# 0xPolygonZero/proof-protocol-decoder

Measured on AMD Instinct MI355X. Metric: txn-proofs/sec (whole node), 256-txn synthetic block, higher is better.
Workload: dtype u64 (Goldilocks field)

## Files before the change

proof_protocol_decoder_amd/csrc/gl.hpp:

```cpp
#pragma once
#include <cstdint>
#include <hip/hip_runtime.h>

#define GL_HD __host__ __device__ __forceinline__

namespace gl {

constexpr uint64_t P = 0xFFFFFFFF00000001ULL;
constexpr uint64_t EPS = 0xFFFFFFFFULL;
constexpr uint64_t GENERATOR = 7;
constexpr uint64_t TWO_ADIC_ROOT = 1753635133440165772ULL;
constexpr uint64_t W = 7;

#if defined(__HIP__)
namespace cc {
typedef uint64_t mask;
__device__ __forceinline__ uint64_t mad_co(uint32_t a, uint32_t b, uint64_t c, mask& co) {
  uint64_t d;
  asm("v_mad_u64_u32 %0, %1, %2, %3, %4" : "=v"(d), "=s"(co) : "v"(a), "v"(b), "v"(c));
  return d;
}
__device__ __forceinline__ uint64_t mad_eps_co(uint32_t a, uint64_t c, mask& co) {
  uint64_t d;
  asm("v_mad_u64_u32 %0, %1, %2, -1, %3" : "=v"(d), "=s"(co) : "v"(a), "v"(c));
  return d;
}
__device__ __forceinline__ uint32_t add_co(uint32_t a, uint32_t b, mask& co) {
  uint32_t d;
  asm("v_add_co_u32_e64 %0, %1, %2, %3" : "=v"(d), "=s"(co) : "v"(a), "v"(b));
  return d;
}
__device__ __forceinline__ uint32_t addc_co(uint32_t a, uint32_t b, mask ci, mask& co) {
  uint32_t d;
  asm("s_nop 1\n\tv_addc_co_u32_e64 %0, %1, %2, %3, %4" : "=v"(d), "=s"(co) : "v"(a), "v"(b), "s"(ci));
  return d;
}
__device__ __forceinline__ uint32_t addc0_co(uint32_t a, mask ci, mask& co) {
  uint32_t d;
  asm("s_nop 1\n\tv_addc_co_u32_e64 %0, %1, %2, 0, %3" : "=v"(d), "=s"(co) : "v"(a), "s"(ci));
  return d;
}
__device__ __forceinline__ uint32_t sub_co(uint32_t a, uint32_t b, mask& co) {
  uint32_t d;
  asm("v_sub_co_u32_e64 %0, %1, %2, %3" : "=v"(d), "=s"(co) : "v"(a), "v"(b));
  return d;
}
__device__ __forceinline__ uint32_t subb_co(uint32_t a, uint32_t b, mask ci, mask& co) {
  uint32_t d;
  asm("s_nop 1\n\tv_subb_co_u32_e64 %0, %1, %2, %3, %4" : "=v"(d), "=s"(co) : "v"(a), "v"(b), "s"(ci));
  return d;
}
__device__ __forceinline__ uint32_t subb0_co(uint32_t a, mask ci, mask& co) {
  uint32_t d;
  asm("s_nop 1\n\tv_subbrev_co_u32_e64 %0, %1, 0, %2, %3" : "=v"(d), "=s"(co) : "v"(a), "s"(ci));
  return d;
}
__device__ __forceinline__ uint32_t sel_eps(mask m) {
  uint32_t d;
  asm("s_nop 1\n\tv_cndmask_b32_e64 %0, 0, -1, %1" : "=v"(d) : "s"(m));
  return d;
}
__device__ __forceinline__ uint64_t mk64(uint32_t lo, uint32_t hi) { return ((uint64_t)hi << 32) | lo; }
#include "gl_cc.inc"
}
#endif
GL_HD uint64_t canon(uint64_t a) {
  return a >= P ? a - P : a;
}

GL_HD uint64_t add(uint64_t a, uint64_t b) {
  uint64_t s = a + b;
  return s < b ? s + EPS : s;
}
GL_HD uint64_t sub(uint64_t a, uint64_t b) {
  uint64_t d = a - b;
  return a < b ? d - EPS : d;
}
GL_HD uint64_t addc(uint64_t a, uint64_t b) {
  uint64_t s = a + b;
  return (s < a || s >= P) ? s - P : s;
}
GL_HD uint64_t subc(uint64_t a, uint64_t b) {
  return a >= b ? a - b : a + (P - b);
}
GL_HD uint64_t negc(uint64_t a) {
  return a ? P - a : 0;
}

GL_HD uint64_t reduce128(uint64_t lo, uint64_t hi) {
  uint64_t hh = hi >> 32, hl = hi & EPS;
  uint64_t t0 = lo - hh;
  if (lo < hh) t0 -= EPS;
  uint64_t t1 = (hl << 32) - hl;
  uint64_t r = t0 + t1;
  return r < t1 ? r + EPS : r;
}

GL_HD void mul_wide(uint64_t a, uint64_t b, uint64_t& lo, uint64_t& hi) {
#if defined(__HIP_DEVICE_COMPILE__)
  uint32_t a0 = (uint32_t)a, a1 = (uint32_t)(a >> 32), b0 = (uint32_t)b, b1 = (uint32_t)(b >> 32);
  uint64_t p00 = (uint64_t)a0 * b0;
  uint64_t mid = (uint64_t)a0 * b1 + (p00 >> 32);
  uint64_t mid2 = (uint64_t)a1 * b0 + (uint32_t)mid;
  hi = (uint64_t)a1 * b1 + (mid >> 32) + (mid2 >> 32);
  lo = (mid2 << 32) | (uint32_t)p00;
#else
  unsigned __int128 x = (unsigned __int128)a * b;
  lo = (uint64_t)x;
  hi = (uint64_t)(x >> 64);
#endif
}

GL_HD uint64_t mul(uint64_t a, uint64_t b) {
#if defined(__HIP_DEVICE_COMPILE__)
  const uint32_t a0 = (uint32_t)a, a1 = (uint32_t)(a >> 32), b0 = (uint32_t)b, b1 = (uint32_t)(b >> 32);
  cc::mask C, c1, c2, c3, cx, bw, bw2, b3;
  const uint64_t P = (uint64_t)a0 * b0;
  const uint64_t M = cc::mad_co(a1, b0, (uint64_t)a0 * b1, C);
  const uint64_t Q = (uint64_t)a1 * b1;
  const uint32_t p1 = cc::add_co((uint32_t)(P >> 32), (uint32_t)M, c1);
  const uint32_t S = cc::addc_co((uint32_t)(M >> 32), (uint32_t)Q, c1, c2);
  const uint32_t K = cc::addc0_co((uint32_t)(Q >> 32), C, cx);
  const uint64_t V = cc::mad_eps_co(S, cc::mk64((uint32_t)P, p1), c3);
  const uint32_t t0 = cc::subb0_co((uint32_t)V, c3, b3);
  const uint32_t t1 = cc::addc0_co((uint32_t)(V >> 32), c3 & ~b3, cx);
  const uint32_t u0 = cc::subb_co(t0, K, c2, bw);
  const uint32_t u1 = cc::subb0_co(t1, bw, bw2);
  const uint32_t r0 = cc::addc0_co(u0, bw2, b3);
  const uint32_t r1 = cc::subb0_co(u1, bw2 & ~b3, cx);
  return cc::mk64(r0, r1);
#else
  uint64_t lo, hi;
  mul_wide(a, b, lo, hi);
  return reduce128(lo, hi);
#endif
}
#if defined(__HIP__)
template <int N>
__device__ __forceinline__ void mul_n(const uint64_t (&a)[N], const uint64_t (&b)[N], uint64_t (&r)[N]) {
  static_assert(N == 3 || N == 4, "groups of 3 or 4");
  uint32_t a1[N], b0[N], t0[N], t1[N], m0[N], m1[N], q0[N], q1[N];
  uint64_t P[N], M[N], Q[N];
  cc::mask C[N], c1[N], c2[N], c3[N], bw[N], bw2[N], b3[N];
#pragma unroll
  for (int i = 0; i < N; i++) {
    const uint32_t a0 = (uint32_t)a[i], b1 = (uint32_t)(b[i] >> 32);
    a1[i] = (uint32_t)(a[i] >> 32);
    b0[i] = (uint32_t)b[i];
    P[i] = (uint64_t)a0 * b0[i];
    M[i] = (uint64_t)a0 * b1;
    Q[i] = (uint64_t)a1[i] * b1;
  }
  cc::mad_co(M, C, a1, b0);
#pragma unroll
  for (int i = 0; i < N; i++) {
    t0[i] = (uint32_t)P[i]; t1[i] = (uint32_t)(P[i] >> 32); m0[i] = (uint32_t)M[i]; m1[i] = (uint32_t)(M[i] >> 32);
    q0[i] = (uint32_t)Q[i]; q1[i] = (uint32_t)(Q[i] >> 32);
  }
  cc::add_co(t1, c1, m0);
  cc::addc_co(m1, c2, q0, c1);
  cc::addc0_cv(q1, C);
#pragma unroll
  for (int i = 0; i < N; i++) P[i] = cc::mk64(t0[i], t1[i]);
  cc::mad_eps_co(P, c3, m1);
#pragma unroll
  for (int i = 0; i < N; i++) { t0[i] = (uint32_t)P[i]; t1[i] = (uint32_t)(P[i] >> 32); }
  cc::subb0_co(t0, b3, c3);
#pragma unroll
  for (int i = 0; i < N; i++) c3[i] &= ~b3[i];
  cc::addc0_cv(t1, c3);
  cc::subb_co(t0, bw, q1, c2);
  cc::subb0_co(t1, bw2, bw);
  cc::addc0_co(t0, b3, bw2);
#pragma unroll
  for (int i = 0; i < N; i++) bw2[i] &= ~b3[i];
  cc::subb0_cv(t1, bw2);
#pragma unroll
  for (int i = 0; i < N; i++) r[i] = cc::mk64(t0[i], t1[i]);
}
#endif
#if defined(__HIP__)
template <int N>
__device__ __forceinline__ void add_n(const uint64_t (&a)[N], const uint64_t (&b)[N], uint64_t (&r)[N]) {
  uint32_t al[N], ah[N], bl[N], bh[N], lo[N], hi[N];
  cc::mask c1[N], c2[N], c3[N];
#pragma unroll
  for (int i = 0; i < N; i++) {
    al[i] = (uint32_t)a[i]; ah[i] = (uint32_t)(a[i] >> 32); bl[i] = (uint32_t)b[i]; bh[i] = (uint32_t)(b[i] >> 32);
  }
  cc::add_co_o(lo, c1, al, bl);
  cc::addc_co_o(hi, c2, ah, bh, c1);
  cc::subb0_co(lo, c3, c2);
#pragma unroll
  for (int i = 0; i < N; i++) c2[i] &= ~c3[i];
  cc::addc0_cv(hi, c2);
#pragma unroll
  for (int i = 0; i < N; i++) r[i] = cc::mk64(lo[i], hi[i]);
}
template <int N>
__device__ __forceinline__ void sub_n(const uint64_t (&a)[N], const uint64_t (&b)[N], uint64_t (&r)[N]) {
  uint32_t al[N], ah[N], bl[N], bh[N], lo[N], hi[N];
  cc::mask b1[N], b2[N], b3[N];
#pragma unroll
  for (int i = 0; i < N; i++) {
    al[i] = (uint32_t)a[i]; ah[i] = (uint32_t)(a[i] >> 32); bl[i] = (uint32_t)b[i]; bh[i] = (uint32_t)(b[i] >> 32);
  }
  cc::sub_co_o(lo, b1, al, bl);
  cc::subb_co_o(hi, b2, ah, bh, b1);
  cc::addc0_co(lo, b3, b2);
#pragma unroll
  for (int i = 0; i < N; i++) b2[i] &= ~b3[i];
  cc::subb0_cv(hi, b2);
#pragma unroll
  for (int i = 0; i < N; i++) r[i] = cc::mk64(lo[i], hi[i]);
}
template <int N>
__device__ __forceinline__ void canon_n(uint64_t (&a)[N]) {
  uint32_t lo[N], hi[N], tl[N], th[N];
  cc::mask k[N], c[N];
#pragma unroll
  for (int i = 0; i < N; i++) {
    lo[i] = (uint32_t)a[i]; hi[i] = (uint32_t)(a[i] >> 32);
  }
  cc::add_m1_co_o(tl, k, lo);
  cc::addc0_co_o(th, c, hi, k);
  cc::sel(lo, tl, c);
  cc::sel(hi, th, c);
#pragma unroll
  for (int i = 0; i < N; i++) a[i] = cc::mk64(lo[i], hi[i]);
}
#endif
#if defined(__HIP__)
struct DotAcc {
  uint64_t p, m, q;
  uint32_t cp, cm, cq;
};
__device__ __forceinline__ DotAcc dot_zero() { return DotAcc{0, 0, 0, 0, 0, 0}; }
__device__ __forceinline__ void dot_mad4(DotAcc (&acc)[4], const uint64_t (&a)[4], const uint64_t (&b)[4]) {
  uint32_t a0[4], a1[4], b0[4], b1[4], cnt[4];
  uint64_t col[4];
  cc::mask c[4], cx[4];
#pragma unroll
  for (int i = 0; i < 4; i++) {
    a0[i] = (uint32_t)a[i]; a1[i] = (uint32_t)(a[i] >> 32); b0[i] = (uint32_t)b[i]; b1[i] = (uint32_t)(b[i] >> 32);
  }
#define BPG_DOT_COL(COL, CNT, X, Y)                                  \
  _Pragma("unroll") for (int i = 0; i < 4; i++) { col[i] = acc[i].COL; cnt[i] = acc[i].CNT; } \
  cc::mad_co(col, c, X, Y);                                           \
  cc::addc0_co(cnt, cx, c);                                           \
  _Pragma("unroll") for (int i = 0; i < 4; i++) { acc[i].COL = col[i]; acc[i].CNT = cnt[i]; }
  BPG_DOT_COL(p, cp, a0, b0)
  BPG_DOT_COL(m, cm, a0, b1)
  BPG_DOT_COL(m, cm, a1, b0)
  BPG_DOT_COL(q, cq, a1, b1)
#undef BPG_DOT_COL
}
GL_HD uint64_t mulc(uint64_t a, uint64_t b);
GL_HD uint64_t addc(uint64_t a, uint64_t b);
__device__ __forceinline__ uint64_t dot_reduce(const DotAcc& d) {
  uint64_t r = canon(d.p);
  r = addc(r, mulc(d.m, (uint64_t)1 << 32));
  r = addc(r, mulc(d.q, EPS));
  r = addc(r, mulc(d.cp, EPS));
  r = subc(r, canon((uint64_t)d.cm));
  r = subc(r, mulc(d.cq, (uint64_t)1 << 32));
  return r;
}
#endif
GL_HD uint64_t sqr(uint64_t a) { return mul(a, a); }
GL_HD uint64_t mulc(uint64_t a, uint64_t b) { return canon(mul(a, b)); }

GL_HD uint64_t pow(uint64_t a, uint64_t e) {
  uint64_t r = 1;
  while (e) {
    if (e & 1) r = mulc(r, a);
    a = mulc(a, a);
    e >>= 1;
  }
  return r;
}
GL_HD uint64_t inv(uint64_t a) {
  auto sq_n = [](uint64_t x, int n) {
    for (int i = 0; i < n; i++) x = mul(x, x);
    return x;
  };
  const uint64_t e1 = a;
  const uint64_t e2 = mul(sq_n(e1, 1), e1);
  const uint64_t e3 = mul(sq_n(e2, 1), e1);
  const uint64_t e6 = mul(sq_n(e3, 3), e3);
  const uint64_t e12 = mul(sq_n(e6, 6), e6);
  const uint64_t e24 = mul(sq_n(e12, 12), e12);
  const uint64_t e30 = mul(sq_n(e24, 6), e6);
  const uint64_t e31 = mul(sq_n(e30, 1), e1);
  const uint64_t hi = sq_n(e31, 1);
  const uint64_t lo = mul(hi, a);
  return mulc(sq_n(hi, 32), lo);
}
GL_HD uint64_t root(unsigned k) {
  uint64_t r = TWO_ADIC_ROOT;
  for (unsigned i = k; i < 32; i++) r = mulc(r, r);
  return r;
}

struct Ext {
  uint64_t c0, c1;
};
GL_HD Ext ext(uint64_t a, uint64_t b = 0) { return Ext{a, b}; }
GL_HD bool eq(Ext a, Ext b) { return a.c0 == b.c0 && a.c1 == b.c1; }
GL_HD Ext add(Ext a, Ext b) { return Ext{addc(a.c0, b.c0), addc(a.c1, b.c1)}; }
GL_HD Ext sub(Ext a, Ext b) { return Ext{subc(a.c0, b.c0), subc(a.c1, b.c1)}; }
GL_HD uint64_t mul7(uint64_t x) {
  const uint64_t p = (uint64_t)(uint32_t)x * 7u;
  const uint64_t m = (x >> 32) * 7u + (p >> 32);
  const uint64_t u = (m << 32) | (uint32_t)p;
  const uint64_t t = u + (m >> 32) * EPS;
  return t < u ? t + EPS : t;
}
GL_HD Ext mul(Ext a, Ext b) {
#if defined(__HIP_DEVICE_COMPILE__)
  const uint64_t x[4] = {a.c0, a.c1, a.c0, a.c1}, y[4] = {b.c0, b.c1, b.c1, b.c0};
  uint64_t r[4];
  mul_n<4>(x, y, r);
  return Ext{addc(canon(r[0]), canon(mul7(r[1]))), addc(canon(r[2]), canon(r[3]))};
#else
  uint64_t c0 = addc(mulc(a.c0, b.c0), mulc(W, mulc(a.c1, b.c1)));
  uint64_t c1 = addc(mulc(a.c0, b.c1), mulc(a.c1, b.c0));
  return Ext{c0, c1};
#endif
}
GL_HD Ext scale(Ext a, uint64_t s) { return Ext{mulc(a.c0, s), mulc(a.c1, s)}; }
GL_HD Ext pow(Ext a, uint64_t e) {
  Ext r = ext(1);
  while (e) {
    if (e & 1) r = mul(r, a);
    a = mul(a, a);
    e >>= 1;
  }
  return r;
}
GL_HD Ext inv(Ext a) {
  uint64_t n = subc(mulc(a.c0, a.c0), mulc(W, mulc(a.c1, a.c1)));
  uint64_t ni = inv(n);
  return Ext{mulc(a.c0, ni), mulc(negc(a.c1), ni)};
}

GL_HD uint32_t bitrev(uint32_t x, unsigned bits) {
#if defined(__HIP_DEVICE_COMPILE__)
  return bits ? (__brev(x) >> (32 - bits)) : 0;
#else
  uint32_t r = 0;
  for (unsigned i = 0; i < bits; i++) r |= ((x >> i) & 1u) << (bits - 1 - i);
  return r;
#endif
}

}
```

proof_protocol_decoder_amd/csrc/gl_cc.inc:

```
__device__ __forceinline__ void mad_co(uint64_t (&x)[3], mask (&co)[3], const uint32_t (&a)[3], const uint32_t (&b)[3]) {
  asm("v_mad_u64_u32 %0, %3, %6, %9, %0\n\tv_mad_u64_u32 %1, %4, %7, %10, %1\n\tv_mad_u64_u32 %2, %5, %8, %11, %2"
      : "+v"(x[0]), "+v"(x[1]), "+v"(x[2]), "=&s"(co[0]), "=&s"(co[1]), "=&s"(co[2])
      : "v"(a[0]), "v"(a[1]), "v"(a[2]), "v"(b[0]), "v"(b[1]), "v"(b[2]));
}
__device__ __forceinline__ void mad_eps_co(uint64_t (&x)[3], mask (&co)[3], const uint32_t (&a)[3]) {
  asm("v_mad_u64_u32 %0, %3, %6, -1, %0\n\tv_mad_u64_u32 %1, %4, %7, -1, %1\n\tv_mad_u64_u32 %2, %5, %8, -1, %2"
      : "+v"(x[0]), "+v"(x[1]), "+v"(x[2]), "=&s"(co[0]), "=&s"(co[1]), "=&s"(co[2])
      : "v"(a[0]), "v"(a[1]), "v"(a[2]));
}
__device__ __forceinline__ void add_co(uint32_t (&x)[3], mask (&co)[3], const uint32_t (&b)[3]) {
  asm("v_add_co_u32_e64 %0, %3, %0, %6\n\tv_add_co_u32_e64 %1, %4, %1, %7\n\tv_add_co_u32_e64 %2, %5, %2, %8"
      : "+v"(x[0]), "+v"(x[1]), "+v"(x[2]), "=&s"(co[0]), "=&s"(co[1]), "=&s"(co[2])
      : "v"(b[0]), "v"(b[1]), "v"(b[2]));
}
__device__ __forceinline__ void addc_co(uint32_t (&x)[3], mask (&co)[3], const uint32_t (&b)[3], const mask (&ci)[3]) {
  asm("v_addc_co_u32_e64 %0, %3, %0, %6, %9\n\tv_addc_co_u32_e64 %1, %4, %1, %7, %10\n\tv_addc_co_u32_e64 %2, %5, %2, %8, %11"
      : "+v"(x[0]), "+v"(x[1]), "+v"(x[2]), "=&s"(co[0]), "=&s"(co[1]), "=&s"(co[2])
      : "v"(b[0]), "v"(b[1]), "v"(b[2]), "s"(ci[0]), "s"(ci[1]), "s"(ci[2]));
}
__device__ __forceinline__ void addc0_co(uint32_t (&x)[3], mask (&co)[3], const mask (&ci)[3]) {
  asm("v_addc_co_u32_e64 %0, %3, %0, 0, %6\n\tv_addc_co_u32_e64 %1, %4, %1, 0, %7\n\tv_addc_co_u32_e64 %2, %5, %2, 0, %8"
      : "+v"(x[0]), "+v"(x[1]), "+v"(x[2]), "=&s"(co[0]), "=&s"(co[1]), "=&s"(co[2])
      : "s"(ci[0]), "s"(ci[1]), "s"(ci[2]));
}
__device__ __forceinline__ void sub_co(uint32_t (&x)[3], mask (&co)[3], const uint32_t (&b)[3]) {
  asm("v_sub_co_u32_e64 %0, %3, %0, %6\n\tv_sub_co_u32_e64 %1, %4, %1, %7\n\tv_sub_co_u32_e64 %2, %5, %2, %8"
      : "+v"(x[0]), "+v"(x[1]), "+v"(x[2]), "=&s"(co[0]), "=&s"(co[1]), "=&s"(co[2])
      : "v"(b[0]), "v"(b[1]), "v"(b[2]));
}
__device__ __forceinline__ void subb_co(uint32_t (&x)[3], mask (&co)[3], const uint32_t (&b)[3], const mask (&ci)[3]) {
  asm("v_subb_co_u32_e64 %0, %3, %0, %6, %9\n\tv_subb_co_u32_e64 %1, %4, %1, %7, %10\n\tv_subb_co_u32_e64 %2, %5, %2, %8, %11"
      : "+v"(x[0]), "+v"(x[1]), "+v"(x[2]), "=&s"(co[0]), "=&s"(co[1]), "=&s"(co[2])
      : "v"(b[0]), "v"(b[1]), "v"(b[2]), "s"(ci[0]), "s"(ci[1]), "s"(ci[2]));
}
__device__ __forceinline__ void subb0_co(uint32_t (&x)[3], mask (&co)[3], const mask (&ci)[3]) {
  asm("v_subbrev_co_u32_e64 %0, %3, 0, %0, %6\n\tv_subbrev_co_u32_e64 %1, %4, 0, %1, %7\n\tv_subbrev_co_u32_e64 %2, %5, 0, %2, %8"
      : "+v"(x[0]), "+v"(x[1]), "+v"(x[2]), "=&s"(co[0]), "=&s"(co[1]), "=&s"(co[2])
      : "s"(ci[0]), "s"(ci[1]), "s"(ci[2]));
}
__device__ __forceinline__ void add_m1_co(uint32_t (&x)[3], mask (&co)[3]) {
  asm("v_add_co_u32_e64 %0, %3, %0, -1\n\tv_add_co_u32_e64 %1, %4, %1, -1\n\tv_add_co_u32_e64 %2, %5, %2, -1"
      : "+v"(x[0]), "+v"(x[1]), "+v"(x[2]), "=&s"(co[0]), "=&s"(co[1]), "=&s"(co[2])
      : );
}
__device__ __forceinline__ void sel(uint32_t (&x)[3], const uint32_t (&b)[3], const mask (&ci)[3]) {
  asm("v_cndmask_b32_e64 %0, %0, %3, %6\n\tv_cndmask_b32_e64 %1, %1, %4, %7\n\tv_cndmask_b32_e64 %2, %2, %5, %8"
      : "+v"(x[0]), "+v"(x[1]), "+v"(x[2])
      : "v"(b[0]), "v"(b[1]), "v"(b[2]), "s"(ci[0]), "s"(ci[1]), "s"(ci[2]));
}
__device__ __forceinline__ void sel_eps(uint32_t (&x)[3], const mask (&ci)[3]) {
  asm("v_cndmask_b32_e64 %0, 0, -1, %3\n\tv_cndmask_b32_e64 %1, 0, -1, %4\n\tv_cndmask_b32_e64 %2, 0, -1, %5"
      : "=&v"(x[0]), "=&v"(x[1]), "=&v"(x[2])
      : "s"(ci[0]), "s"(ci[1]), "s"(ci[2]));
}
__device__ __forceinline__ void addc0_cv(uint32_t (&x)[3], const mask (&ci)[3]) {
  asm("v_addc_co_u32_e64 %0, vcc, %0, 0, %3\n\tv_addc_co_u32_e64 %1, vcc, %1, 0, %4\n\tv_addc_co_u32_e64 %2, vcc, %2, 0, %5"
      : "+v"(x[0]), "+v"(x[1]), "+v"(x[2])
      : "s"(ci[0]), "s"(ci[1]), "s"(ci[2]) : "vcc");
}
__device__ __forceinline__ void addc_cv(uint32_t (&x)[3], const uint32_t (&b)[3], const mask (&ci)[3]) {
  asm("v_addc_co_u32_e64 %0, vcc, %0, %3, %6\n\tv_addc_co_u32_e64 %1, vcc, %1, %4, %7\n\tv_addc_co_u32_e64 %2, vcc, %2, %5, %8"
      : "+v"(x[0]), "+v"(x[1]), "+v"(x[2])
      : "v"(b[0]), "v"(b[1]), "v"(b[2]), "s"(ci[0]), "s"(ci[1]), "s"(ci[2]) : "vcc");
}
__device__ __forceinline__ void subb0_cv(uint32_t (&x)[3], const mask (&ci)[3]) {
  asm("v_subbrev_co_u32_e64 %0, vcc, 0, %0, %3\n\tv_subbrev_co_u32_e64 %1, vcc, 0, %1, %4\n\tv_subbrev_co_u32_e64 %2, vcc, 0, %2, %5"
      : "+v"(x[0]), "+v"(x[1]), "+v"(x[2])
      : "s"(ci[0]), "s"(ci[1]), "s"(ci[2]) : "vcc");
}
__device__ __forceinline__ void mad_eps_cv(uint64_t (&x)[3], const uint32_t (&a)[3]) {
  asm("v_mad_u64_u32 %0, vcc, %3, -1, %0\n\tv_mad_u64_u32 %1, vcc, %4, -1, %1\n\tv_mad_u64_u32 %2, vcc, %5, -1, %2"
      : "+v"(x[0]), "+v"(x[1]), "+v"(x[2])
      : "v"(a[0]), "v"(a[1]), "v"(a[2]) : "vcc");
}
__device__ __forceinline__ void sel_one(uint32_t (&x)[3], const mask (&ci)[3]) {
  asm("v_cndmask_b32_e64 %0, %0, 1, %3\n\tv_cndmask_b32_e64 %1, %1, 1, %4\n\tv_cndmask_b32_e64 %2, %2, 1, %5"
      : "+v"(x[0]), "+v"(x[1]), "+v"(x[2])
      : "s"(ci[0]), "s"(ci[1]), "s"(ci[2]));
}
__device__ __forceinline__ void add_co_o(uint32_t (&x)[3], mask (&co)[3], const uint32_t (&a)[3], const uint32_t (&b)[3]) {
  asm("v_add_co_u32_e64 %0, %3, %6, %9\n\tv_add_co_u32_e64 %1, %4, %7, %10\n\tv_add_co_u32_e64 %2, %5, %8, %11"
      : "=&v"(x[0]), "=&v"(x[1]), "=&v"(x[2]), "=&s"(co[0]), "=&s"(co[1]), "=&s"(co[2])
      : "v"(a[0]), "v"(a[1]), "v"(a[2]), "v"(b[0]), "v"(b[1]), "v"(b[2]));
}
__device__ __forceinline__ void addc_co_o(uint32_t (&x)[3], mask (&co)[3], const uint32_t (&a)[3], const uint32_t (&b)[3], const mask (&ci)[3]) {
  asm("v_addc_co_u32_e64 %0, %3, %6, %9, %12\n\tv_addc_co_u32_e64 %1, %4, %7, %10, %13\n\tv_addc_co_u32_e64 %2, %5, %8, %11, %14"
      : "=&v"(x[0]), "=&v"(x[1]), "=&v"(x[2]), "=&s"(co[0]), "=&s"(co[1]), "=&s"(co[2])
      : "v"(a[0]), "v"(a[1]), "v"(a[2]), "v"(b[0]), "v"(b[1]), "v"(b[2]), "s"(ci[0]), "s"(ci[1]), "s"(ci[2]));
}
__device__ __forceinline__ void sub_co_o(uint32_t (&x)[3], mask (&co)[3], const uint32_t (&a)[3], const uint32_t (&b)[3]) {
  asm("v_sub_co_u32_e64 %0, %3, %6, %9\n\tv_sub_co_u32_e64 %1, %4, %7, %10\n\tv_sub_co_u32_e64 %2, %5, %8, %11"
      : "=&v"(x[0]), "=&v"(x[1]), "=&v"(x[2]), "=&s"(co[0]), "=&s"(co[1]), "=&s"(co[2])
      : "v"(a[0]), "v"(a[1]), "v"(a[2]), "v"(b[0]), "v"(b[1]), "v"(b[2]));
}
__device__ __forceinline__ void subb_co_o(uint32_t (&x)[3], mask (&co)[3], const uint32_t (&a)[3], const uint32_t (&b)[3], const mask (&ci)[3]) {
  asm("v_subb_co_u32_e64 %0, %3, %6, %9, %12\n\tv_subb_co_u32_e64 %1, %4, %7, %10, %13\n\tv_subb_co_u32_e64 %2, %5, %8, %11, %14"
      : "=&v"(x[0]), "=&v"(x[1]), "=&v"(x[2]), "=&s"(co[0]), "=&s"(co[1]), "=&s"(co[2])
      : "v"(a[0]), "v"(a[1]), "v"(a[2]), "v"(b[0]), "v"(b[1]), "v"(b[2]), "s"(ci[0]), "s"(ci[1]), "s"(ci[2]));
}
__device__ __forceinline__ void add_m1_co_o(uint32_t (&x)[3], mask (&co)[3], const uint32_t (&a)[3]) {
  asm("v_add_co_u32_e64 %0, %3, %6, -1\n\tv_add_co_u32_e64 %1, %4, %7, -1\n\tv_add_co_u32_e64 %2, %5, %8, -1"
      : "=&v"(x[0]), "=&v"(x[1]), "=&v"(x[2]), "=&s"(co[0]), "=&s"(co[1]), "=&s"(co[2])
      : "v"(a[0]), "v"(a[1]), "v"(a[2]));
}
__device__ __forceinline__ void addc0_co_o(uint32_t (&x)[3], mask (&co)[3], const uint32_t (&a)[3], const mask (&ci)[3]) {
  asm("v_addc_co_u32_e64 %0, %3, %6, 0, %9\n\tv_addc_co_u32_e64 %1, %4, %7, 0, %10\n\tv_addc_co_u32_e64 %2, %5, %8, 0, %11"
      : "=&v"(x[0]), "=&v"(x[1]), "=&v"(x[2]), "=&s"(co[0]), "=&s"(co[1]), "=&s"(co[2])
      : "v"(a[0]), "v"(a[1]), "v"(a[2]), "s"(ci[0]), "s"(ci[1]), "s"(ci[2]));
}
__device__ __forceinline__ void mad_co(uint64_t (&x)[4], mask (&co)[4], const uint32_t (&a)[4], const uint32_t (&b)[4]) {
  asm("v_mad_u64_u32 %0, %4, %8, %12, %0\n\tv_mad_u64_u32 %1, %5, %9, %13, %1\n\tv_mad_u64_u32 %2, %6, %10, %14, %2\n\tv_mad_u64_u32 %3, %7, %11, %15, %3"
      : "+v"(x[0]), "+v"(x[1]), "+v"(x[2]), "+v"(x[3]), "=&s"(co[0]), "=&s"(co[1]), "=&s"(co[2]), "=&s"(co[3])
      : "v"(a[0]), "v"(a[1]), "v"(a[2]), "v"(a[3]), "v"(b[0]), "v"(b[1]), "v"(b[2]), "v"(b[3]));
}
__device__ __forceinline__ void mad_eps_co(uint64_t (&x)[4], mask (&co)[4], const uint32_t (&a)[4]) {
  asm("v_mad_u64_u32 %0, %4, %8, -1, %0\n\tv_mad_u64_u32 %1, %5, %9, -1, %1\n\tv_mad_u64_u32 %2, %6, %10, -1, %2\n\tv_mad_u64_u32 %3, %7, %11, -1, %3"
      : "+v"(x[0]), "+v"(x[1]), "+v"(x[2]), "+v"(x[3]), "=&s"(co[0]), "=&s"(co[1]), "=&s"(co[2]), "=&s"(co[3])
      : "v"(a[0]), "v"(a[1]), "v"(a[2]), "v"(a[3]));
}
__device__ __forceinline__ void add_co(uint32_t (&x)[4], mask (&co)[4], const uint32_t (&b)[4]) {
  asm("v_add_co_u32_e64 %0, %4, %0, %8\n\tv_add_co_u32_e64 %1, %5, %1, %9\n\tv_add_co_u32_e64 %2, %6, %2, %10\n\tv_add_co_u32_e64 %3, %7, %3, %11"
      : "+v"(x[0]), "+v"(x[1]), "+v"(x[2]), "+v"(x[3]), "=&s"(co[0]), "=&s"(co[1]), "=&s"(co[2]), "=&s"(co[3])
      : "v"(b[0]), "v"(b[1]), "v"(b[2]), "v"(b[3]));
}
__device__ __forceinline__ void addc_co(uint32_t (&x)[4], mask (&co)[4], const uint32_t (&b)[4], const mask (&ci)[4]) {
  asm("v_addc_co_u32_e64 %0, %4, %0, %8, %12\n\tv_addc_co_u32_e64 %1, %5, %1, %9, %13\n\tv_addc_co_u32_e64 %2, %6, %2, %10, %14\n\tv_addc_co_u32_e64 %3, %7, %3, %11, %15"
      : "+v"(x[0]), "+v"(x[1]), "+v"(x[2]), "+v"(x[3]), "=&s"(co[0]), "=&s"(co[1]), "=&s"(co[2]), "=&s"(co[3])
      : "v"(b[0]), "v"(b[1]), "v"(b[2]), "v"(b[3]), "s"(ci[0]), "s"(ci[1]), "s"(ci[2]), "s"(ci[3]));
}
__device__ __forceinline__ void addc0_co(uint32_t (&x)[4], mask (&co)[4], const mask (&ci)[4]) {
  asm("v_addc_co_u32_e64 %0, %4, %0, 0, %8\n\tv_addc_co_u32_e64 %1, %5, %1, 0, %9\n\tv_addc_co_u32_e64 %2, %6, %2, 0, %10\n\tv_addc_co_u32_e64 %3, %7, %3, 0, %11"
      : "+v"(x[0]), "+v"(x[1]), "+v"(x[2]), "+v"(x[3]), "=&s"(co[0]), "=&s"(co[1]), "=&s"(co[2]), "=&s"(co[3])
      : "s"(ci[0]), "s"(ci[1]), "s"(ci[2]), "s"(ci[3]));
}
__device__ __forceinline__ void sub_co(uint32_t (&x)[4], mask (&co)[4], const uint32_t (&b)[4]) {
  asm("v_sub_co_u32_e64 %0, %4, %0, %8\n\tv_sub_co_u32_e64 %1, %5, %1, %9\n\tv_sub_co_u32_e64 %2, %6, %2, %10\n\tv_sub_co_u32_e64 %3, %7, %3, %11"
      : "+v"(x[0]), "+v"(x[1]), "+v"(x[2]), "+v"(x[3]), "=&s"(co[0]), "=&s"(co[1]), "=&s"(co[2]), "=&s"(co[3])
      : "v"(b[0]), "v"(b[1]), "v"(b[2]), "v"(b[3]));
}
__device__ __forceinline__ void subb_co(uint32_t (&x)[4], mask (&co)[4], const uint32_t (&b)[4], const mask (&ci)[4]) {
  asm("v_subb_co_u32_e64 %0, %4, %0, %8, %12\n\tv_subb_co_u32_e64 %1, %5, %1, %9, %13\n\tv_subb_co_u32_e64 %2, %6, %2, %10, %14\n\tv_subb_co_u32_e64 %3, %7, %3, %11, %15"
      : "+v"(x[0]), "+v"(x[1]), "+v"(x[2]), "+v"(x[3]), "=&s"(co[0]), "=&s"(co[1]), "=&s"(co[2]), "=&s"(co[3])
      : "v"(b[0]), "v"(b[1]), "v"(b[2]), "v"(b[3]), "s"(ci[0]), "s"(ci[1]), "s"(ci[2]), "s"(ci[3]));
}
__device__ __forceinline__ void subb0_co(uint32_t (&x)[4], mask (&co)[4], const mask (&ci)[4]) {
  asm("v_subbrev_co_u32_e64 %0, %4, 0, %0, %8\n\tv_subbrev_co_u32_e64 %1, %5, 0, %1, %9\n\tv_subbrev_co_u32_e64 %2, %6, 0, %2, %10\n\tv_subbrev_co_u32_e64 %3, %7, 0, %3, %11"
      : "+v"(x[0]), "+v"(x[1]), "+v"(x[2]), "+v"(x[3]), "=&s"(co[0]), "=&s"(co[1]), "=&s"(co[2]), "=&s"(co[3])
      : "s"(ci[0]), "s"(ci[1]), "s"(ci[2]), "s"(ci[3]));
}
__device__ __forceinline__ void add_m1_co(uint32_t (&x)[4], mask (&co)[4]) {
  asm("v_add_co_u32_e64 %0, %4, %0, -1\n\tv_add_co_u32_e64 %1, %5, %1, -1\n\tv_add_co_u32_e64 %2, %6, %2, -1\n\tv_add_co_u32_e64 %3, %7, %3, -1"
      : "+v"(x[0]), "+v"(x[1]), "+v"(x[2]), "+v"(x[3]), "=&s"(co[0]), "=&s"(co[1]), "=&s"(co[2]), "=&s"(co[3])
      : );
}
__device__ __forceinline__ void sel(uint32_t (&x)[4], const uint32_t (&b)[4], const mask (&ci)[4]) {
  asm("v_cndmask_b32_e64 %0, %0, %4, %8\n\tv_cndmask_b32_e64 %1, %1, %5, %9\n\tv_cndmask_b32_e64 %2, %2, %6, %10\n\tv_cndmask_b32_e64 %3, %3, %7, %11"
      : "+v"(x[0]), "+v"(x[1]), "+v"(x[2]), "+v"(x[3])
      : "v"(b[0]), "v"(b[1]), "v"(b[2]), "v"(b[3]), "s"(ci[0]), "s"(ci[1]), "s"(ci[2]), "s"(ci[3]));
}
__device__ __forceinline__ void sel_eps(uint32_t (&x)[4], const mask (&ci)[4]) {
  asm("v_cndmask_b32_e64 %0, 0, -1, %4\n\tv_cndmask_b32_e64 %1, 0, -1, %5\n\tv_cndmask_b32_e64 %2, 0, -1, %6\n\tv_cndmask_b32_e64 %3, 0, -1, %7"
      : "=&v"(x[0]), "=&v"(x[1]), "=&v"(x[2]), "=&v"(x[3])
      : "s"(ci[0]), "s"(ci[1]), "s"(ci[2]), "s"(ci[3]));
}
__device__ __forceinline__ void addc0_cv(uint32_t (&x)[4], const mask (&ci)[4]) {
  asm("v_addc_co_u32_e64 %0, vcc, %0, 0, %4\n\tv_addc_co_u32_e64 %1, vcc, %1, 0, %5\n\tv_addc_co_u32_e64 %2, vcc, %2, 0, %6\n\tv_addc_co_u32_e64 %3, vcc, %3, 0, %7"
      : "+v"(x[0]), "+v"(x[1]), "+v"(x[2]), "+v"(x[3])
      : "s"(ci[0]), "s"(ci[1]), "s"(ci[2]), "s"(ci[3]) : "vcc");
}
__device__ __forceinline__ void addc_cv(uint32_t (&x)[4], const uint32_t (&b)[4], const mask (&ci)[4]) {
  asm("v_addc_co_u32_e64 %0, vcc, %0, %4, %8\n\tv_addc_co_u32_e64 %1, vcc, %1, %5, %9\n\tv_addc_co_u32_e64 %2, vcc, %2, %6, %10\n\tv_addc_co_u32_e64 %3, vcc, %3, %7, %11"
      : "+v"(x[0]), "+v"(x[1]), "+v"(x[2]), "+v"(x[3])
      : "v"(b[0]), "v"(b[1]), "v"(b[2]), "v"(b[3]), "s"(ci[0]), "s"(ci[1]), "s"(ci[2]), "s"(ci[3]) : "vcc");
}
__device__ __forceinline__ void subb0_cv(uint32_t (&x)[4], const mask (&ci)[4]) {
  asm("v_subbrev_co_u32_e64 %0, vcc, 0, %0, %4\n\tv_subbrev_co_u32_e64 %1, vcc, 0, %1, %5\n\tv_subbrev_co_u32_e64 %2, vcc, 0, %2, %6\n\tv_subbrev_co_u32_e64 %3, vcc, 0, %3, %7"
      : "+v"(x[0]), "+v"(x[1]), "+v"(x[2]), "+v"(x[3])
      : "s"(ci[0]), "s"(ci[1]), "s"(ci[2]), "s"(ci[3]) : "vcc");
}
__device__ __forceinline__ void mad_eps_cv(uint64_t (&x)[4], const uint32_t (&a)[4]) {
  asm("v_mad_u64_u32 %0, vcc, %4, -1, %0\n\tv_mad_u64_u32 %1, vcc, %5, -1, %1\n\tv_mad_u64_u32 %2, vcc, %6, -1, %2\n\tv_mad_u64_u32 %3, vcc, %7, -1, %3"
      : "+v"(x[0]), "+v"(x[1]), "+v"(x[2]), "+v"(x[3])
      : "v"(a[0]), "v"(a[1]), "v"(a[2]), "v"(a[3]) : "vcc");
}
__device__ __forceinline__ void sel_one(uint32_t (&x)[4], const mask (&ci)[4]) {
  asm("v_cndmask_b32_e64 %0, %0, 1, %4\n\tv_cndmask_b32_e64 %1, %1, 1, %5\n\tv_cndmask_b32_e64 %2, %2, 1, %6\n\tv_cndmask_b32_e64 %3, %3, 1, %7"
      : "+v"(x[0]), "+v"(x[1]), "+v"(x[2]), "+v"(x[3])
      : "s"(ci[0]), "s"(ci[1]), "s"(ci[2]), "s"(ci[3]));
}
__device__ __forceinline__ void add_co_o(uint32_t (&x)[4], mask (&co)[4], const uint32_t (&a)[4], const uint32_t (&b)[4]) {
  asm("v_add_co_u32_e64 %0, %4, %8, %12\n\tv_add_co_u32_e64 %1, %5, %9, %13\n\tv_add_co_u32_e64 %2, %6, %10, %14\n\tv_add_co_u32_e64 %3, %7, %11, %15"
      : "=&v"(x[0]), "=&v"(x[1]), "=&v"(x[2]), "=&v"(x[3]), "=&s"(co[0]), "=&s"(co[1]), "=&s"(co[2]), "=&s"(co[3])
      : "v"(a[0]), "v"(a[1]), "v"(a[2]), "v"(a[3]), "v"(b[0]), "v"(b[1]), "v"(b[2]), "v"(b[3]));
}
__device__ __forceinline__ void addc_co_o(uint32_t (&x)[4], mask (&co)[4], const uint32_t (&a)[4], const uint32_t (&b)[4], const mask (&ci)[4]) {
  asm("v_addc_co_u32_e64 %0, %4, %8, %12, %16\n\tv_addc_co_u32_e64 %1, %5, %9, %13, %17\n\tv_addc_co_u32_e64 %2, %6, %10, %14, %18\n\tv_addc_co_u32_e64 %3, %7, %11, %15, %19"
      : "=&v"(x[0]), "=&v"(x[1]), "=&v"(x[2]), "=&v"(x[3]), "=&s"(co[0]), "=&s"(co[1]), "=&s"(co[2]), "=&s"(co[3])
      : "v"(a[0]), "v"(a[1]), "v"(a[2]), "v"(a[3]), "v"(b[0]), "v"(b[1]), "v"(b[2]), "v"(b[3]), "s"(ci[0]), "s"(ci[1]), "s"(ci[2]), "s"(ci[3]));
}
__device__ __forceinline__ void sub_co_o(uint32_t (&x)[4], mask (&co)[4], const uint32_t (&a)[4], const uint32_t (&b)[4]) {
  asm("v_sub_co_u32_e64 %0, %4, %8, %12\n\tv_sub_co_u32_e64 %1, %5, %9, %13\n\tv_sub_co_u32_e64 %2, %6, %10, %14\n\tv_sub_co_u32_e64 %3, %7, %11, %15"
      : "=&v"(x[0]), "=&v"(x[1]), "=&v"(x[2]), "=&v"(x[3]), "=&s"(co[0]), "=&s"(co[1]), "=&s"(co[2]), "=&s"(co[3])
      : "v"(a[0]), "v"(a[1]), "v"(a[2]), "v"(a[3]), "v"(b[0]), "v"(b[1]), "v"(b[2]), "v"(b[3]));
}
__device__ __forceinline__ void subb_co_o(uint32_t (&x)[4], mask (&co)[4], const uint32_t (&a)[4], const uint32_t (&b)[4], const mask (&ci)[4]) {
  asm("v_subb_co_u32_e64 %0, %4, %8, %12, %16\n\tv_subb_co_u32_e64 %1, %5, %9, %13, %17\n\tv_subb_co_u32_e64 %2, %6, %10, %14, %18\n\tv_subb_co_u32_e64 %3, %7, %11, %15, %19"
      : "=&v"(x[0]), "=&v"(x[1]), "=&v"(x[2]), "=&v"(x[3]), "=&s"(co[0]), "=&s"(co[1]), "=&s"(co[2]), "=&s"(co[3])
      : "v"(a[0]), "v"(a[1]), "v"(a[2]), "v"(a[3]), "v"(b[0]), "v"(b[1]), "v"(b[2]), "v"(b[3]), "s"(ci[0]), "s"(ci[1]), "s"(ci[2]), "s"(ci[3]));
}
__device__ __forceinline__ void add_m1_co_o(uint32_t (&x)[4], mask (&co)[4], const uint32_t (&a)[4]) {
  asm("v_add_co_u32_e64 %0, %4, %8, -1\n\tv_add_co_u32_e64 %1, %5, %9, -1\n\tv_add_co_u32_e64 %2, %6, %10, -1\n\tv_add_co_u32_e64 %3, %7, %11, -1"
      : "=&v"(x[0]), "=&v"(x[1]), "=&v"(x[2]), "=&v"(x[3]), "=&s"(co[0]), "=&s"(co[1]), "=&s"(co[2]), "=&s"(co[3])
      : "v"(a[0]), "v"(a[1]), "v"(a[2]), "v"(a[3]));
}
__device__ __forceinline__ void addc0_co_o(uint32_t (&x)[4], mask (&co)[4], const uint32_t (&a)[4], const mask (&ci)[4]) {
  asm("v_addc_co_u32_e64 %0, %4, %8, 0, %12\n\tv_addc_co_u32_e64 %1, %5, %9, 0, %13\n\tv_addc_co_u32_e64 %2, %6, %10, 0, %14\n\tv_addc_co_u32_e64 %3, %7, %11, 0, %15"
      : "=&v"(x[0]), "=&v"(x[1]), "=&v"(x[2]), "=&v"(x[3]), "=&s"(co[0]), "=&s"(co[1]), "=&s"(co[2]), "=&s"(co[3])
      : "v"(a[0]), "v"(a[1]), "v"(a[2]), "v"(a[3]), "s"(ci[0]), "s"(ci[1]), "s"(ci[2]), "s"(ci[3]));
}
```

proof_protocol_decoder_amd/csrc/ntt.hip:

```cpp
#include <atomic>
#include <map>
#include <mutex>
#include <tuple>
#include <cstring>
#include <memory>
#include "common.hpp"
#include "gl.hpp"
#include "mx_arith.cuh"

namespace {

constexpr uint32_t LOG_BLK_MAX = 14;

template <int N>
__device__ __forceinline__ void mul_group(uint64_t (&x)[16], const int (&idx)[4], const uint64_t (&d)[4], const uint64_t (&w)[4]) {
  if constexpr (N == 4) {
    uint64_t r[4];
    gl::mul_n<4>(d, w, r);
#pragma unroll
    for (int i = 0; i < 4; i++) x[idx[i]] = r[i];
  } else if constexpr (N == 3) {
    const uint64_t d3[3] = {d[0], d[1], d[2]}, w3[3] = {w[0], w[1], w[2]};
    uint64_t r[3];
    gl::mul_n<3>(d3, w3, r);
#pragma unroll
    for (int i = 0; i < 3; i++) x[idx[i]] = r[i];
  } else {
#pragma unroll
    for (int i = 0; i < N; i++) x[idx[i]] = gl::mul(d[i], w[i]);
  }
}

template <int LOGR, bool J0 = false>
__device__ __forceinline__ void dif_butterflies(uint64_t (&x)[1 << LOGR], const uint64_t* __restrict__ tw,
                                                uint32_t j, uint32_t log_sub, uint32_t tw_shift) {
  constexpr int R = 1 << LOGR, NB = R / 2;
#pragma unroll
  for (int s = 0; s < LOGR; s++) {
    const int half = R >> (s + 1);
    if constexpr (NB % 4 == 0 && J0 && LOGR == 4) {
      uint64_t dd[NB];
#pragma unroll
      for (int k0 = 0; k0 < NB; k0 += 4) {
        uint64_t a[4], b[4], d[4], r[4];
#pragma unroll
        for (int i = 0; i < 4; i++) {
          const int k = k0 + i, m = (k / half) * 2 * half + (k % half);
          a[i] = x[m];
          b[i] = x[m + half];
        }
        gl::canon_n<4>(b);
        gl::add_n<4>(a, b, r);
        gl::sub_n<4>(a, b, d);
#pragma unroll
        for (int i = 0; i < 4; i++) {
          const int k = k0 + i, m = (k / half) * 2 * half + (k % half);
          x[m] = r[i];
          dd[k] = d[i];
        }
      }
      int cnt = 0;
      int idx[4] = {0, 0, 0, 0};
      uint64_t dv[4] = {0, 0, 0, 0}, wv[4] = {0, 0, 0, 0};
      uint64_t xx[16];
#pragma unroll
      for (int i = 0; i < 16; i++) xx[i] = x[i];
#pragma unroll
      for (int k = 0; k < NB; k++) {
        const int m = (k / half) * 2 * half + (k % half), e = m & (half - 1);
        if (e == 0) {
          xx[m + half] = dd[k];
        } else {
          idx[cnt] = m + half;
          dv[cnt] = dd[k];
          wv[cnt] = tw[(uint32_t)e << (tw_shift + s)];
          cnt++;
          if (cnt == 4) {
            mul_group<4>(xx, idx, dv, wv);
            cnt = 0;
          }
        }
      }
      if (cnt == 3) mul_group<3>(xx, idx, dv, wv);
      else if (cnt == 2) mul_group<2>(xx, idx, dv, wv);
      else if (cnt == 1) mul_group<1>(xx, idx, dv, wv);
#pragma unroll
      for (int i = 0; i < 16; i++) x[i] = xx[i];
    } else if constexpr (NB % 4 == 0) {
#pragma unroll
      for (int k0 = 0; k0 < NB; k0 += 4) {
        uint64_t a[4], b[4], d[4], w[4], r[4];
#pragma unroll
        for (int i = 0; i < 4; i++) {
          const int k = k0 + i, m = (k / half) * 2 * half + (k % half);
          const uint32_t p = j + ((uint32_t)(m & (half - 1)) << log_sub);
          w[i] = tw[p << (tw_shift + s)];
          a[i] = x[m];
          b[i] = x[m + half];
        }
        gl::canon_n<4>(b);
        gl::add_n<4>(a, b, r);
        gl::sub_n<4>(a, b, d);
#pragma unroll
        for (int i = 0; i < 4; i++) {
          const int k = k0 + i, m = (k / half) * 2 * half + (k % half);
          x[m] = r[i];
        }
        gl::mul_n<4>(d, w, r);
#pragma unroll
        for (int i = 0; i < 4; i++) {
          const int k = k0 + i, m = (k / half) * 2 * half + (k % half);
          x[m + half] = r[i];
        }
        if constexpr (LOGR >= 4) __builtin_amdgcn_sched_barrier(0);
      }
    } else {
#pragma unroll
      for (int m = 0; m < R; m++) {
        if (m & half) continue;
        const uint64_t a = x[m], b = gl::canon(x[m + half]);
        x[m] = gl::add(a, b);
        if (J0 && (m & (half - 1)) == 0) {
          x[m + half] = gl::sub(a, b);
        } else {
          const uint32_t p = j + ((uint32_t)(m & (half - 1)) << log_sub);
          x[m + half] = gl::mul(gl::sub(a, b), tw[p << (tw_shift + s)]);
        }
      }
    }
  }
}
template <int LOGR, bool J0 = false>
__device__ __forceinline__ void dit_butterflies(uint64_t (&x)[1 << LOGR], const uint64_t* __restrict__ tw,
                                                uint32_t j, uint32_t log_sub, uint32_t tw_shift) {
  constexpr int R = 1 << LOGR, NB = R / 2;
#pragma unroll
  for (int s = 0; s < LOGR; s++) {
    const int step = 1 << s;
    if constexpr (NB % 4 == 0 && J0 && LOGR == 4) {
      uint64_t xx[16];
#pragma unroll
      for (int i = 0; i < 16; i++) xx[i] = x[i];
      int cnt = 0;
      int idx[4] = {0, 0, 0, 0};
      uint64_t dv[4] = {0, 0, 0, 0}, wv[4] = {0, 0, 0, 0};
#pragma unroll
      for (int k = 0; k < NB; k++) {
        const int m = (k / step) * 2 * step + (k % step), e = m & (step - 1);
        if (e != 0) {
          idx[cnt] = m + step;
          dv[cnt] = x[m + step];
          wv[cnt] = tw[(uint32_t)e << (tw_shift + (LOGR - 1 - s))];
          cnt++;
          if (cnt == 4) {
            mul_group<4>(xx, idx, dv, wv);
            cnt = 0;
          }
        }
      }
      if (cnt == 3) mul_group<3>(xx, idx, dv, wv);
      else if (cnt == 2) mul_group<2>(xx, idx, dv, wv);
      else if (cnt == 1) mul_group<1>(xx, idx, dv, wv);
#pragma unroll
      for (int k0 = 0; k0 < NB; k0 += 4) {
        uint64_t a[4], r[4], hi[4], lo[4];
#pragma unroll
        for (int i = 0; i < 4; i++) {
          const int k = k0 + i, m = (k / step) * 2 * step + (k % step);
          a[i] = xx[m];
          r[i] = xx[m + step];
        }
        gl::canon_n<4>(r);
        gl::add_n<4>(a, r, hi);
        gl::sub_n<4>(a, r, lo);
#pragma unroll
        for (int i = 0; i < 4; i++) {
          const int k = k0 + i, m = (k / step) * 2 * step + (k % step);
          x[m] = hi[i];
          x[m + step] = lo[i];
        }
      }
    } else if constexpr (NB % 4 == 0) {
#pragma unroll
      for (int k0 = 0; k0 < NB; k0 += 4) {
        uint64_t a[4], v[4], w[4], r[4], hi[4], lo[4];
#pragma unroll
        for (int i = 0; i < 4; i++) {
          const int k = k0 + i, m = (k / step) * 2 * step + (k % step);
          const uint32_t p = j + ((uint32_t)(m & (step - 1)) << log_sub);
          w[i] = tw[p << (tw_shift + (LOGR - 1 - s))];
          v[i] = x[m + step];
          a[i] = x[m];
        }
        gl::mul_n<4>(v, w, r);
        gl::canon_n<4>(r);
        gl::add_n<4>(a, r, hi);
        gl::sub_n<4>(a, r, lo);
#pragma unroll
        for (int i = 0; i < 4; i++) {
          const int k = k0 + i, m = (k / step) * 2 * step + (k % step);
          x[m] = hi[i];
          x[m + step] = lo[i];
        }
        if constexpr (LOGR >= 4) __builtin_amdgcn_sched_barrier(0);
      }
    } else {
#pragma unroll
      for (int m = 0; m < R; m++) {
        if (m & step) continue;
        const uint32_t p = j + ((uint32_t)(m & (step - 1)) << log_sub);
        const uint64_t a = x[m];
        const uint64_t t = (J0 && (m & (step - 1)) == 0) ? gl::canon(x[m + step])
                                                         : gl::mulc(x[m + step], tw[p << (tw_shift + (LOGR - 1 - s))]);
        x[m] = gl::add(a, t);
        x[m + step] = gl::sub(a, t);
      }
    }
  }
}

template <int LOGR, bool DIF>
__device__ __forceinline__ void lds_pass(uint64_t* buf, uint32_t log_blk, uint32_t span_log,
                                         const uint64_t* __restrict__ tw) {
  constexpr int R = 1 << LOGR;
  const uint32_t log_sub = span_log - LOGR, sub_mask = (1u << log_sub) - 1;
  const uint32_t n_q = 1u << (log_blk - LOGR);
  for (uint32_t q = threadIdx.x; q < n_q; q += blockDim.x) {
    const uint32_t j = q & sub_mask, blk = q >> log_sub;
    const uint32_t base = (blk << span_log) + j;
    uint64_t x[R];
#pragma unroll
    for (int m = 0; m < R; m++) x[m] = buf[base + ((uint32_t)m << log_sub)];
    if (DIF) dif_butterflies<LOGR>(x, tw, j, log_sub, log_blk - span_log);
    else dit_butterflies<LOGR>(x, tw, j, log_sub, log_blk - span_log);
#pragma unroll
    for (int m = 0; m < R; m++) buf[base + ((uint32_t)m << log_sub)] = x[m];
  }
}

struct LdsNttArgs {
  const uint64_t* in;
  uint64_t in_stride;
  uint64_t* out;
  uint64_t out_stride;
  uint64_t out_coset_stride;
  const uint64_t* tw;
  const uint64_t* scale;
  uint64_t out_scalar;
  uint32_t log_blk;
  uint32_t log_n_total;
};

template <bool DIF>
__global__ void __launch_bounds__(1024) ntt_lds_kernel(LdsNttArgs a) {
  if (gridDim.x * gridDim.y * gridDim.z <= 64) __builtin_amdgcn_s_setprio(3);
  extern __shared__ uint64_t buf[];
  const uint32_t n = 1u << a.log_blk;
  const uint64_t off = (uint64_t)blockIdx.x << a.log_blk;
  const uint64_t* src = a.in + blockIdx.y * a.in_stride + off;
  uint64_t* dst = a.out + blockIdx.y * a.out_stride + blockIdx.z * a.out_coset_stride + off;
  if (!DIF && a.scale) {
    const uint64_t* sc = a.scale + ((uint64_t)blockIdx.z << a.log_n_total) + off;
    for (uint32_t i = threadIdx.x; i < n; i += blockDim.x) buf[i] = gl::mulc(src[i], sc[i]);
  } else {
    for (uint32_t i = threadIdx.x; i < n; i += blockDim.x) buf[i] = src[i];
  }
  __syncthreads();
  const uint32_t rem = a.log_blk % 3;
  if (DIF) {
    uint32_t span = a.log_blk;
    for (; span >= 3 && span > rem; span -= 3) {
      lds_pass<3, true>(buf, a.log_blk, span, a.tw);
      __syncthreads();
    }
    if (rem == 1) lds_pass<1, true>(buf, a.log_blk, 1, a.tw);
    else if (rem == 2) lds_pass<2, true>(buf, a.log_blk, 2, a.tw);
    if (rem) __syncthreads();
  } else {
    if (rem == 1) lds_pass<1, false>(buf, a.log_blk, 1, a.tw);
    else if (rem == 2) lds_pass<2, false>(buf, a.log_blk, 2, a.tw);
    if (rem) __syncthreads();
    for (uint32_t span = rem + 3; span <= a.log_blk; span += 3) {
      lds_pass<3, false>(buf, a.log_blk, span, a.tw);
      __syncthreads();
    }
  }
  if (DIF && a.out_scalar != 1) {
    for (uint32_t i = threadIdx.x; i < n; i += blockDim.x) dst[i] = gl::mulc(buf[i], a.out_scalar);
  } else {
    for (uint32_t i = threadIdx.x; i < n; i += blockDim.x) dst[i] = gl::canon(buf[i]);
  }
}

template <int L>
__device__ __forceinline__ uint32_t swz(uint32_t i) {
  uint32_t x;
  if (L == 14) x = (((i >> 6) & 7u) << 2) ^ ((i >> 9) & 31u);
  else if (L == 13) x = (((i >> 5) & 15u) << 1) ^ ((i >> 9) & 15u);
  else x = (((i >> 8) & 1u) << 4) ^ ((i >> 7) & 1u) ^ (((i >> 9) & 7u) << 1);
  return i ^ x;
}
__device__ __forceinline__ uint32_t insert4(uint32_t t, uint32_t m, uint32_t b) {
  return ((t >> b) << (b + 4)) | (m << b) | (t & ((1u << b) - 1));
}
template <int R, int SH, bool CONTIG, bool DIF>
__device__ __forceinline__ void sub_butterflies(uint64_t (&x)[16], const uint64_t* __restrict__ tw, uint32_t j,
                                                uint32_t j_step_log, uint32_t log_sub, uint32_t tw_shift) {
  constexpr int G = 16 >> R;
#pragma unroll
  for (int g = 0; g < G; g++) {
    uint64_t y[1 << R];
#pragma unroll
    for (int u = 0; u < (1 << R); u++) y[u] = CONTIG ? x[(g << R) + u] : x[g + (u << SH)];
    const uint32_t jj = CONTIG ? 0u : j + ((uint32_t)g << j_step_log);
    if (DIF) dif_butterflies<R, CONTIG>(y, tw, jj, log_sub, tw_shift);
    else dit_butterflies<R, CONTIG>(y, tw, jj, log_sub, tw_shift);
#pragma unroll
    for (int u = 0; u < (1 << R); u++) {
      if (CONTIG) x[(g << R) + u] = y[u];
      else x[g + (u << SH)] = y[u];
    }
  }
}

struct Ntt16Args {
  const uint64_t* in;
  uint64_t in_stride;
  uint64_t* out;
  uint64_t out_stride, out_coset_stride;
  const uint64_t* tw;
  const uint64_t* scale;
  uint64_t out_scalar;
  uint32_t log_n_total, n_cosets, n_units;
  const uint64_t* tw_top;
};


template <int L, int F>
__global__ void __launch_bounds__((1 << L) / 16) ntt16_dif_kernel(Ntt16Args a) {
  if (gridDim.x * gridDim.y * gridDim.z <= 64) __builtin_amdgcn_s_setprio(3);
  extern __shared__ uint64_t buf[];
  constexpr uint32_t T = (1u << L) / 16;
  constexpr int RT = (L % 4 == 0) ? 4 : (L % 4);
  const uint32_t t = threadIdx.x;
  const uint64_t* src;
  uint64_t* dst;
  uint64_t x[16];
  if (F) {
    const uint32_t id = blockIdx.x, k = id >> 3, h = k & 1, unit = (k >> 1) * 8 + (id & 7);
    if (unit >= a.n_units) return;
    const uint32_t log_bpc = a.log_n_total - (L + 1);
    const uint32_t col = unit >> log_bpc, blk = unit & ((1u << log_bpc) - 1);
    const uint64_t off = (uint64_t)blk << (L + 1);
    src = a.in + col * a.in_stride + off;
    dst = a.out + col * a.out_stride + off + ((uint64_t)h << L);
#pragma unroll
    for (int m0 = 0; m0 < 16; m0 += 4) {
      uint64_t lo[4], hi[4], r[4];
#pragma unroll
      for (int i = 0; i < 4; i++) {
        lo[i] = src[(m0 + i) * T + t];
        hi[i] = src[(m0 + i) * T + t + (1u << L)];
      }
      gl::canon_n<4>(hi);
      if (h == 0) {
        gl::add_n<4>(lo, hi, r);
      } else {
        uint64_t d[4], w[4];
        gl::sub_n<4>(lo, hi, d);
#pragma unroll
        for (int i = 0; i < 4; i++) w[i] = a.tw_top[(m0 + i) * T + t];
        gl::mul_n<4>(d, w, r);
      }
#pragma unroll
      for (int i = 0; i < 4; i++) x[m0 + i] = r[i];
    }
  } else {
    const uint64_t off = (uint64_t)blockIdx.x << L;
    src = a.in + blockIdx.y * a.in_stride + off;
    dst = a.out + blockIdx.y * a.out_stride + off;
#pragma unroll
    for (int m = 0; m < 16; m++) x[m] = src[m * T + t];
  }
  dif_butterflies<4>(x, a.tw, t, L - 4, 0);
#pragma unroll
  for (int m = 0; m < 16; m++) buf[swz<L>(m * T + t)] = x[m];
  __syncthreads();
#pragma unroll
  for (int b = L - 8; b > 0; b -= 4) {
#pragma unroll
    for (int m = 0; m < 16; m++) x[m] = buf[swz<L>(insert4(t, m, b))];
    dif_butterflies<4>(x, a.tw, t & ((1u << b) - 1), b, L - (b + 4));
#pragma unroll
    for (int m = 0; m < 16; m++) buf[swz<L>(insert4(t, m, b))] = x[m];
    __syncthreads();
  }
  const uint32_t base = gl::bitrev(t, L - 4) << 4;
#pragma unroll
  for (int m = 0; m < 16; m++) x[m] = buf[swz<L>(base | m)];
  sub_butterflies<RT, 0, true, true>(x, a.tw, 0, 0, 0, L - RT);
#pragma unroll
  for (int m = 0; m < 16; m++) buf[swz<L>(base | m)] = x[m];
  __syncthreads();
  if (a.out_scalar != 1) {
#pragma unroll
    for (int m0 = 0; m0 < 16; m0 += 4) {
      uint64_t v[4], w[4], r[4];
#pragma unroll
      for (int i = 0; i < 4; i++) {
        v[i] = buf[swz<L>((m0 + i) * T + t)];
        w[i] = a.out_scalar;
      }
      gl::mul_n<4>(v, w, r);
      gl::canon_n<4>(r);
#pragma unroll
      for (int i = 0; i < 4; i++) dst[(m0 + i) * T + t] = r[i];
    }
  } else {
#pragma unroll
    for (int m0 = 0; m0 < 16; m0 += 4) {
      uint64_t v[4];
#pragma unroll
      for (int i = 0; i < 4; i++) v[i] = buf[swz<L>((m0 + i) * T + t)];
      gl::canon_n<4>(v);
#pragma unroll
      for (int i = 0; i < 4; i++) dst[(m0 + i) * T + t] = v[i];
    }
  }
}

template <int L, int F>
__global__ void __launch_bounds__((1 << L) / 16) __attribute__((amdgpu_waves_per_eu(4, 8))) ntt16_dit_kernel(Ntt16Args a) {
  if (gridDim.x <= 64) __builtin_amdgcn_s_setprio(3);
  extern __shared__ uint64_t buf[];
  constexpr uint32_t T = (1u << L) / 16;
  constexpr int RT = (L % 4 == 0) ? 4 : (L % 4);
  const uint32_t id = blockIdx.x, k = id >> 3;
  const uint32_t per = a.n_cosets << F;
  const uint32_t ch = k % per, coset = ch >> F, h = F ? (ch & 1) : 0, unit = (k / per) * 8 + (id & 7);
  if (unit >= a.n_units) return;
  const uint32_t log_bpc = a.log_n_total - (L + F);
  const uint32_t col = unit >> log_bpc, blk = unit & ((1u << log_bpc) - 1);
  const uint32_t t = threadIdx.x;
  const uint64_t off = (uint64_t)blk << (L + F);
  const uint64_t* src = a.in + col * a.in_stride + off;
  const uint64_t* tw = a.tw;
  uint64_t x[16];
  const uint32_t base = gl::bitrev(t, L - 4) << 4;
  if (F) {
    const ulonglong2* src2 = reinterpret_cast<const ulonglong2*>(src);
    const ulonglong2* sc2 = a.scale ? reinterpret_cast<const ulonglong2*>(a.scale + ((uint64_t)coset << a.log_n_total) + off) : nullptr;
    constexpr uint32_t BR4[16] = {0, 8, 4, 12, 2, 10, 6, 14, 1, 9, 5, 13, 3, 11, 7, 15};
#pragma unroll
    for (int m0 = 0; m0 < 16; m0 += 4) {
      uint64_t c0[4], c1[4], r[4];
#pragma unroll
      for (int i = 0; i < 4; i++) {
        const ulonglong2 c = src2[(m0 + i) * T + t];
        c0[i] = c.x;
        c1[i] = c.y;
      }
      if (sc2) {
        uint64_t s0[4], s1[4], p0[4], p1[4];
#pragma unroll
        for (int i = 0; i < 4; i++) {
          const ulonglong2 sc = sc2[(m0 + i) * T + t];
          s0[i] = sc.x;
          s1[i] = sc.y;
        }
        gl::mul_n<4>(c0, s0, p0);
        gl::mul_n<4>(c1, s1, p1);
        gl::canon_n<4>(p1);
#pragma unroll
        for (int i = 0; i < 4; i++) { c0[i] = p0[i]; c1[i] = p1[i]; }
      } else {
        gl::canon_n<4>(c1);
      }
      if (h == 0) {
        gl::add_n<4>(c0, c1, r);
      } else {
        uint64_t d[4], w[4];
        gl::sub_n<4>(c0, c1, d);
#pragma unroll
        for (int i = 0; i < 4; i++) w[i] = a.tw_top[base | BR4[m0 + i]];
        gl::mul_n<4>(d, w, r);
      }
#pragma unroll
      for (int i = 0; i < 4; i++) buf[swz<L>((m0 + i) * T + t)] = r[i];
    }
  } else if (a.scale) {
    const uint64_t* sc = a.scale + ((uint64_t)coset << a.log_n_total) + off;
#pragma unroll
    for (int m0 = 0; m0 < 16; m0 += 4) {
      uint64_t v[4], w[4], r[4];
#pragma unroll
      for (int i = 0; i < 4; i++) {
        v[i] = src[(m0 + i) * T + t];
        w[i] = sc[(m0 + i) * T + t];
      }
      gl::mul_n<4>(v, w, r);
#pragma unroll
      for (int i = 0; i < 4; i++) buf[swz<L>((m0 + i) * T + t)] = r[i];
    }
  } else {
#pragma unroll
    for (int m = 0; m < 16; m++) buf[swz<L>(m * T + t)] = src[m * T + t];
  }
  __syncthreads();
#pragma unroll
  for (int m = 0; m < 16; m++) x[m] = buf[swz<L>(base | m)];
  dit_butterflies<4, true>(x, tw, 0, 0, L - 4);
#pragma unroll
  for (int m = 0; m < 16; m++) buf[swz<L>(base | m)] = x[m];
  __syncthreads();
#pragma unroll
  for (int b = 4; b + 4 <= L - RT; b += 4) {
#pragma unroll
    for (int m = 0; m < 16; m++) x[m] = buf[swz<L>(insert4(t, m, b))];
    dit_butterflies<4>(x, tw, t & ((1u << b) - 1), b, L - (b + 4));
#pragma unroll
    for (int m = 0; m < 16; m++) buf[swz<L>(insert4(t, m, b))] = x[m];
    __syncthreads();
  }
  uint32_t t2 = t;
  asm volatile("" : "+v"(t2));
#pragma unroll
  for (int m = 0; m < 16; m++) x[m] = buf[swz<L>(m * T + t2)];
  sub_butterflies<RT, 4 - RT, false, false>(x, tw, t2, L - 4, L - RT, 0);
  uint64_t* dst = a.out + col * a.out_stride + coset * a.out_coset_stride + off;
#pragma unroll
  for (int m0 = 0; m0 < 16; m0 += 4) {
    uint64_t v[4] = {x[m0], x[m0 + 1], x[m0 + 2], x[m0 + 3]};
    gl::canon_n<4>(v);
#pragma unroll
    for (int i = 0; i < 4; i++) {
      if (F) dst[2 * ((m0 + i) * T + t2) + h] = v[i];
      else dst[(m0 + i) * T + t2] = v[i];
    }
  }
}

template <int L>
__global__ void __launch_bounds__((1 << L) / 16) __attribute__((amdgpu_waves_per_eu(4, 4)))
ntt16_dit_persist_kernel(Ntt16Args a, uint32_t n_items) {
  extern __shared__ uint64_t buf[];
  constexpr uint32_t T = (1u << L) / 16;
  constexpr int RT = (L % 4 == 0) ? 4 : (L % 4);
  const uint32_t t = threadIdx.x;
  const uint32_t log_bpc = a.log_n_total - L;
  const uint64_t* tw = a.tw;
  auto source_of = [&](uint32_t id) -> const uint64_t* {
    const uint32_t k = id >> 3, unit = (k / a.n_cosets) * 8 + (id & 7);
    if (id >= n_items || unit >= a.n_units) return nullptr;
    const uint32_t col = unit >> log_bpc, blk = unit & ((1u << log_bpc) - 1);
    return a.in + col * a.in_stride + ((uint64_t)blk << L);
  };
  uint64_t xn[16];
  {
    const uint64_t* s0 = source_of(blockIdx.x);
    if (s0) {
#pragma unroll
      for (int m = 0; m < 16; m++) xn[m] = s0[m * T + t];
    }
  }
  for (uint32_t id = blockIdx.x; id < n_items; id += gridDim.x) {
    const uint32_t k = id >> 3, coset = k % a.n_cosets, unit = (k / a.n_cosets) * 8 + (id & 7);
    const uint64_t* next_src = source_of(id + gridDim.x);
    uint32_t ta = t, tb = t, tc = t;
    asm volatile("" : "+v"(ta));
    if (unit >= a.n_units) {
      if (next_src) {
#pragma unroll
        for (int m = 0; m < 16; m++) xn[m] = next_src[m * T + t];
      }
      continue;
    }
    const uint32_t col = unit >> log_bpc, blk = unit & ((1u << log_bpc) - 1);
    const uint64_t off = (uint64_t)blk << L;
    if (a.scale) {
      const uint64_t* sc = a.scale + ((uint64_t)coset << a.log_n_total) + off;
#pragma unroll
      for (int m0 = 0; m0 < 16; m0 += 4) {
        uint64_t v[4], w[4], r[4];
#pragma unroll
        for (int i = 0; i < 4; i++) {
          v[i] = xn[m0 + i];
          w[i] = sc[(m0 + i) * T + ta];
        }
        gl::mul_n<4>(v, w, r);
#pragma unroll
        for (int i = 0; i < 4; i++) buf[swz<L>((m0 + i) * T + ta)] = r[i];
      }
    } else {
#pragma unroll
      for (int m = 0; m < 16; m++) buf[swz<L>(m * T + ta)] = xn[m];
    }
    __syncthreads();
    asm volatile("" : "+v"(tb));
    const uint32_t base = gl::bitrev(tb, L - 4) << 4;
    uint64_t x[16];
#pragma unroll
    for (int m = 0; m < 16; m++) x[m] = buf[swz<L>(base | m)];
    dit_butterflies<4, true>(x, tw, 0, 0, L - 4);
#pragma unroll
    for (int m = 0; m < 16; m++) buf[swz<L>(base | m)] = x[m];
    __syncthreads();
#pragma unroll
    for (int b = 4; b + 4 <= L - RT; b += 4) {
      asm volatile("" : "+v"(tc));
#pragma unroll
      for (int m = 0; m < 16; m++) x[m] = buf[swz<L>(insert4(tc, m, b))];
      dit_butterflies<4>(x, tw, tc & ((1u << b) - 1), b, L - (b + 4));
#pragma unroll
      for (int m = 0; m < 16; m++) buf[swz<L>(insert4(tc, m, b))] = x[m];
      __syncthreads();
    }
    uint32_t t2 = t;
    asm volatile("" : "+v"(t2));
    if (next_src) {
#pragma unroll
      for (int m = 0; m < 16; m++) xn[m] = next_src[m * T + t2];
    }
#pragma unroll
    for (int m = 0; m < 16; m++) x[m] = buf[swz<L>(m * T + t2)];
    sub_butterflies<RT, 4 - RT, false, false>(x, tw, t2, L - 4, L - RT, 0);
    uint64_t* dst = a.out + col * a.out_stride + coset * a.out_coset_stride + off;
#pragma unroll
    for (int m0 = 0; m0 < 16; m0 += 4) {
      uint64_t v[4] = {x[m0], x[m0 + 1], x[m0 + 2], x[m0 + 3]};
      gl::canon_n<4>(v);
#pragma unroll
      for (int i = 0; i < 4; i++) dst[(m0 + i) * T + t2] = v[i];
    }
  }
}

#include "ntt_mx.cuh"

template <int LOGR, bool DIF>
__global__ void __launch_bounds__(256)
ntt_global_pass_kernel(const uint64_t* in, uint64_t in_stride, uint64_t* out, uint64_t out_stride,
                       uint64_t coset_stride, uint32_t log_n, uint32_t span_log,
                       const uint64_t* __restrict__ tw) {
  constexpr int R = 1 << LOGR;
  const uint32_t log_sub = span_log - LOGR;
  const uint32_t q = blockIdx.x * blockDim.x + threadIdx.x;
  if (q >= (1u << (log_n - LOGR))) return;
  const uint32_t j = q & ((1u << log_sub) - 1), blk = q >> log_sub;
  const uint64_t base = ((uint64_t)blk << span_log) + j;
  const uint64_t* src = in + blockIdx.y * in_stride + blockIdx.z * coset_stride + base;
  uint64_t* dst = out + blockIdx.y * out_stride + blockIdx.z * coset_stride + base;
  uint64_t x[R];
#pragma unroll
  for (int m = 0; m < R; m++) x[m] = src[(uint64_t)m << log_sub];
  if (DIF) dif_butterflies<LOGR>(x, tw, j, log_sub, log_n - span_log);
  else dit_butterflies<LOGR>(x, tw, j, log_sub, log_n - span_log);
  if constexpr (R % 4 == 0) {
#pragma unroll
    for (int m0 = 0; m0 < R; m0 += 4) {
      uint64_t v[4] = {x[m0], x[m0 + 1], x[m0 + 2], x[m0 + 3]};
      gl::canon_n<4>(v);
#pragma unroll
      for (int i = 0; i < 4; i++) dst[(uint64_t)(m0 + i) << log_sub] = v[i];
    }
  } else {
#pragma unroll
    for (int m = 0; m < R; m++) dst[(uint64_t)m << log_sub] = gl::canon(x[m]);
  }
}


template <int A, bool DIF>
__global__ void __launch_bounds__(1 << A)
ntt_tile_kernel(const uint64_t* in, uint64_t in_stride, uint64_t* out, uint64_t out_stride, uint64_t coset_stride,
                uint32_t log_n, uint32_t span_log, const uint64_t* __restrict__ tw) {
  constexpr int R = 1 << A, B = A - 4, R1 = 1 << B, G = 16 / R1;
  __shared__ uint64_t tile[R * 16];
  const uint32_t log_s = span_log - A;
  const uint32_t tiles_per_blk = 1u << (log_s - 4);
  const uint32_t blk = blockIdx.x / tiles_per_blk, s0 = (blockIdx.x % tiles_per_blk) << 4;
  const uint32_t s = threadIdx.x & 15, hi = threadIdx.x >> 4;
  const uint64_t base = ((uint64_t)blk << span_log) + s0 + s;
  const uint64_t* src = in + blockIdx.y * in_stride + blockIdx.z * coset_stride + base;
  uint64_t* dst = out + blockIdx.y * out_stride + blockIdx.z * coset_stride + base;
  const uint32_t j16 = (hi << log_s) + s0 + s;
  uint64_t x[16];
  if (DIF) {
#pragma unroll
    for (int m = 0; m < 16; m++) x[m] = src[(uint64_t)(hi + m * (R / 16)) << log_s];
    dif_butterflies<4>(x, tw, j16, span_log - 4, log_n - span_log);
#pragma unroll
    for (int m = 0; m < 16; m++) tile[(hi + m * (R / 16)) * 16 + s] = x[m];
    __syncthreads();
#pragma unroll
    for (int m = 0; m < 16; m++) x[m] = tile[(hi * 16 + m) * 16 + s];
#pragma unroll
    for (int g = 0; g < G; g++) {
      uint64_t y[R1];
#pragma unroll
      for (int u = 0; u < R1; u++) y[u] = x[g * R1 + u];
      dif_butterflies<B>(y, tw, s0 + s, log_s, log_n - span_log + 4);
#pragma unroll
      for (int u = 0; u < R1; u++) x[g * R1 + u] = y[u];
    }
#pragma unroll
    for (int m0 = 0; m0 < 16; m0 += 4) {
      uint64_t v[4] = {x[m0], x[m0 + 1], x[m0 + 2], x[m0 + 3]};
      gl::canon_n<4>(v);
#pragma unroll
      for (int i = 0; i < 4; i++) dst[(uint64_t)(hi * 16 + m0 + i) << log_s] = v[i];
    }
  } else {
#pragma unroll
    for (int m = 0; m < 16; m++) x[m] = src[(uint64_t)(hi * 16 + m) << log_s];
#pragma unroll
    for (int g = 0; g < G; g++) {
      uint64_t y[R1];
#pragma unroll
      for (int u = 0; u < R1; u++) y[u] = x[g * R1 + u];
      dit_butterflies<B>(y, tw, s0 + s, log_s, log_n - span_log + 4);
#pragma unroll
      for (int u = 0; u < R1; u++) x[g * R1 + u] = y[u];
    }
#pragma unroll
    for (int m = 0; m < 16; m++) tile[(hi * 16 + m) * 16 + s] = x[m];
    __syncthreads();
#pragma unroll
    for (int m = 0; m < 16; m++) x[m] = tile[(hi + m * (R / 16)) * 16 + s];
    dit_butterflies<4>(x, tw, j16, span_log - 4, log_n - span_log);
#pragma unroll
    for (int m0 = 0; m0 < 16; m0 += 4) {
      uint64_t v[4] = {x[m0], x[m0 + 1], x[m0 + 2], x[m0 + 3]};
      gl::canon_n<4>(v);
#pragma unroll
      for (int i = 0; i < 4; i++) dst[(uint64_t)(hi + (m0 + i) * (R / 16)) << log_s] = v[i];
    }
  }
}

__global__ void twiddle_table_kernel(uint64_t* out, uint32_t count, uint64_t w) {
  uint32_t e = blockIdx.x * blockDim.x + threadIdx.x;
  if (e < count) out[e] = gl::pow(w, e);
}
__global__ void coset_scale_table_kernel(uint64_t* out, uint32_t log_n, uint32_t rate_bits, uint64_t w_m,
                                         int inverse) {
  uint32_t pos = blockIdx.x * blockDim.x + threadIdx.x;
  if (pos >= (1u << log_n)) return;
  uint32_t t = blockIdx.y;
  uint64_t g = gl::mulc(gl::GENERATOR, gl::pow(w_m, t));
  if (inverse) g = gl::inv(g);
  out[((uint64_t)t << log_n) + pos] = gl::pow(g, gl::bitrev(pos, log_n));
}
__global__ void bitrev_permute_kernel(uint64_t* cols, uint64_t stride, uint32_t log_n) {
  uint32_t i = blockIdx.x * blockDim.x + threadIdx.x;
  if (i >= (1u << log_n)) return;
  uint32_t j = gl::bitrev(i, log_n);
  if (i < j) {
    uint64_t* c = cols + blockIdx.y * stride;
    uint64_t a = c[i], b = c[j];
    c[i] = b;
    c[j] = a;
  }
}

struct TableKey {
  int dev, kind;
  uint32_t log_n, rate_bits;
  bool operator<(const TableKey& o) const {
    return std::tie(dev, kind, log_n, rate_bits) < std::tie(o.dev, o.kind, o.log_n, o.rate_bits);
  }
};
std::mutex g_table_mu;
std::map<TableKey, uint64_t*> g_tables;

}

namespace bpg {

int get_table(int kind, uint32_t log_n, uint32_t rate_bits, const uint64_t** out) {
  int dev = 0;
  BPG_HIP(hipGetDevice(&dev));
  std::lock_guard<std::mutex> lk(g_table_mu);
  TableKey key{dev, kind, log_n, kind >= 2 ? rate_bits : 0};
  auto it = g_tables.find(key);
  if (it != g_tables.end()) {
    *out = it->second;
    return BP_OK;
  }
  uint64_t* d = nullptr;
  if (kind >= 2) {
    uint64_t count = (uint64_t)1 << (log_n + rate_bits);
    BPG_HIP(hipMalloc(&d, count * 8));
    dim3 grid(ceil_div((uint64_t)1 << log_n, 256), 1u << rate_bits);
    coset_scale_table_kernel<<<grid, 256, 0, 0>>>(d, log_n, rate_bits, gl::root(log_n + rate_bits), kind == 3);
  } else {
    uint32_t count = log_n ? (1u << (log_n - 1)) : 1;
    BPG_HIP(hipMalloc(&d, (uint64_t)count * 8));
    uint64_t w = gl::root(log_n);
    if (kind == 1) w = gl::inv(w);
    twiddle_table_kernel<<<ceil_div(count, 256), 256, 0, 0>>>(d, count, w);
  }
  BPG_LAUNCH_CHECK();
  BPG_HIP(hipStreamSynchronize(0));
  g_tables[key] = d;
  *out = d;
  return BP_OK;
}

bool device_loaded();
static std::atomic<int> g_ntt_mx{3};
static bool use_ntt_mx(uint32_t log_blk, bool dit) {
  const int m = g_ntt_mx.load(std::memory_order_relaxed);
  if (m == 3) return log_blk == 13 && !device_loaded();
  if (m == 4) return !dit && log_blk <= 13;
  if (m == 5) return dit && log_blk <= 13;
  return m == 2 || (m == 1 && log_blk <= 13);
}
static std::mutex g_mx_mu;
static std::map<std::tuple<int, int, int>, mxn::Tables*> g_mx_tabs;
static std::atomic<int> g_mx_wg_per_cu{0};
static uint32_t mx_grid(uint32_t items, uint32_t log_blk) {
  static const int cus = [] {
    int dev = 0, n = 256;
    if (hipGetDevice(&dev) == hipSuccess) (void)hipDeviceGetAttribute(&n, hipDeviceAttributeMultiprocessorCount, dev);
    return n > 0 ? n : 256;
  }();
  int per = g_mx_wg_per_cu.load(std::memory_order_relaxed);
  if (per <= 0) per = log_blk == 12 ? 2 : 1;
  const uint32_t resident = ((uint32_t)cus * per + 7) / 8 * 8;
  return items < resident ? items : resident;
}
static int get_mx_tables(int kind, bool inverse, const mxn::Tables** out) {
  int dev = 0;
  BPG_HIP(hipGetDevice(&dev));
  std::lock_guard<std::mutex> lk(g_mx_mu);
  const auto key = std::make_tuple(dev, kind, inverse ? 1 : 0);
  auto it = g_mx_tabs.find(key);
  if (it != g_mx_tabs.end()) {
    *out = it->second;
    return BP_OK;
  }
  auto host = std::make_unique<mxn::Tables>();
  mxn::build_tables(*host, kind, inverse);
  mxn::Tables* d = nullptr;
  BPG_HIP(hipMalloc(&d, sizeof(mxn::Tables)));
  BPG_HIP(hipMemcpy(d, host.get(), sizeof(mxn::Tables), hipMemcpyHostToDevice));
  g_mx_tabs[key] = d;
  *out = d;
  return BP_OK;
}

struct NttPlan {
  uint32_t log_blk;
  uint32_t tile_bits;
  uint32_t n_reg;
  uint32_t reg_bits[4];
};
static NttPlan plan_ntt(uint32_t log_n) {
  NttPlan p{};
  if (log_n <= LOG_BLK_MAX) { p.log_blk = log_n; return p; }
  if (log_n <= 17) { p.log_blk = log_n <= 16 ? 12 : 13; p.n_reg = 1; p.reg_bits[0] = log_n - p.log_blk; return p; }
  if (log_n <= 20) { p.log_blk = 12; p.tile_bits = log_n - 12; return p; }
  if (log_n <= 22) { p.log_blk = log_n - 8; p.tile_bits = 8; return p; }
  p.log_blk = 14; p.tile_bits = 8;
  uint32_t left = log_n - 22;
  p.n_reg = (left + 3) / 4;
  for (uint32_t i = 0; i < p.n_reg; i++) {
    const uint32_t k = (left + (p.n_reg - i) - 1) / (p.n_reg - i);
    p.reg_bits[i] = k;
    left -= k;
  }
  return p;
}
static uint32_t pick_log_blk(uint32_t log_n) { return plan_ntt(log_n).log_blk; }

static std::atomic<int> g_ntt_persist{0};
static std::atomic<int> g_ntt_persist_wgs{256};
static std::atomic<int> g_ntt_split{0};
static bool use_split(uint32_t log_blk, uint64_t workgroups, const void* src, const void* dst, bool dit) {
  const int mode = g_ntt_split.load(std::memory_order_relaxed);
  if (mode == 1 || log_blk < 13 || src == dst) return false;
  if (mode == 2) return true;
  if (dit) return mode == 3 && log_blk == 13 && workgroups < 512;
  return log_blk == 14 || workgroups < 512;
}

static uint32_t lds_threads(uint32_t log_blk) {
  uint32_t t = log_blk >= 3 ? (1u << (log_blk - 3)) : 1;
  return t < 64 ? 64 : (t > 1024 ? 1024 : t);
}

template <bool DIF>
static int launch_global_passes(const uint64_t* in, uint64_t in_stride, uint64_t* out, uint64_t out_stride,
                                uint64_t coset_stride, uint32_t n_cols, uint32_t n_cosets, uint32_t log_n,
                                uint32_t log_blk, const uint64_t* tw, hipStream_t st) {
  const NttPlan p = plan_ntt(log_n);
  uint32_t spans[8], bits[8], tiled[8], cnt = 0;
  uint32_t span = log_n;
  for (uint32_t i = 0; i < p.n_reg; i++) { spans[cnt] = span; bits[cnt] = p.reg_bits[i]; tiled[cnt] = 0; cnt++; span -= p.reg_bits[i]; }
  if (p.tile_bits) { spans[cnt] = span; bits[cnt] = p.tile_bits; tiled[cnt] = 1; cnt++; span -= p.tile_bits; }
  if (span != log_blk || log_blk != p.log_blk) return fail(BP_ERR_DEVICE, "NTT plan mismatch (log_n=%u)", log_n);
  for (uint32_t idx = 0; idx < cnt; idx++) {
    const uint32_t i = DIF ? idx : cnt - 1 - idx;
    const uint64_t* src = (idx == 0) ? in : out;
    const uint64_t src_stride = (idx == 0) ? in_stride : out_stride;
    if (tiled[i]) {
      const dim3 grid(1u << (log_n - bits[i] - 4), n_cols, n_cosets);
      switch (bits[i]) {
        case 6: ntt_tile_kernel<6, DIF><<<grid, 64, 0, st>>>(src, src_stride, out, out_stride, coset_stride, log_n, spans[i], tw); break;
        case 7: ntt_tile_kernel<7, DIF><<<grid, 128, 0, st>>>(src, src_stride, out, out_stride, coset_stride, log_n, spans[i], tw); break;
        default: ntt_tile_kernel<8, DIF><<<grid, 256, 0, st>>>(src, src_stride, out, out_stride, coset_stride, log_n, spans[i], tw); break;
      }
    } else {
      const dim3 grid(ceil_div((uint64_t)1 << (log_n - bits[i]), 256), n_cols, n_cosets);
      switch (bits[i]) {
        case 1: ntt_global_pass_kernel<1, DIF><<<grid, 256, 0, st>>>(src, src_stride, out, out_stride, coset_stride, log_n, spans[i], tw); break;
        case 2: ntt_global_pass_kernel<2, DIF><<<grid, 256, 0, st>>>(src, src_stride, out, out_stride, coset_stride, log_n, spans[i], tw); break;
        case 3: ntt_global_pass_kernel<3, DIF><<<grid, 256, 0, st>>>(src, src_stride, out, out_stride, coset_stride, log_n, spans[i], tw); break;
        case 4: ntt_global_pass_kernel<4, DIF><<<grid, 256, 0, st>>>(src, src_stride, out, out_stride, coset_stride, log_n, spans[i], tw); break;
        default: return fail(BP_ERR_DEVICE, "NTT plan asks for a %u-stage register pass", bits[i]);
      }
    }
    BPG_LAUNCH_CHECK();
  }
  return BP_OK;
}

int intt_nat2br(const uint64_t* in, uint64_t in_stride, uint64_t* out, uint64_t out_stride, uint32_t log_n,
                uint32_t n_cols, bool inverse, hipStream_t st) {
  if (n_cols == 0) return BP_OK;
  const uint32_t log_blk = pick_log_blk(log_n);
  const uint64_t *tw_n = nullptr, *tw_b = nullptr;
  int rc;
  if ((rc = get_table(inverse ? 1 : 0, log_blk, 0, &tw_b))) return rc;
  const uint64_t* src = in;
  uint64_t src_stride = in_stride;
  if (log_n > LOG_BLK_MAX) {
    if ((rc = get_table(inverse ? 1 : 0, log_n, 0, &tw_n))) return rc;
    if ((rc = launch_global_passes<true>(in, in_stride, out, out_stride, 0, n_cols, 1, log_n, log_blk, tw_n, st))) return rc;
    src = out;
    src_stride = out_stride;
  }
  if (log_blk >= 12) {
    Ntt16Args b{};
    b.in = src; b.in_stride = src_stride; b.out = out; b.out_stride = out_stride; b.out_coset_stride = 0;
    b.tw = tw_b; b.scale = nullptr; b.out_scalar = inverse ? gl::inv((uint64_t)1 << log_n) : 1;
    b.log_n_total = log_n; b.n_cosets = 1; b.n_units = 0;
    KernelTimer kt(PROF_INTT_DIF, st, 16.0 * (double)n_cols * (double)((uint64_t)1 << log_n));
    if (use_ntt_mx(log_blk, false)) {
      const mxn::Tables* tab = nullptr;
      if ((rc = get_mx_tables(0, inverse, &tab))) return rc;
      b.n_units = n_cols << (log_n - log_blk);
      const uint32_t g = mx_grid(b.n_units, log_blk);
      if (log_blk == 12) mxn::ntt_mx_dif_kernel<0><<<g, 256, (8u << 12) + 4 * mxn::C_LDS_WORDS, st>>>(b, tab);
      else if (log_blk == 13) mxn::ntt_mx_dif_kernel<1><<<g, 512, (8u << 13) + 4 * mxn::C_LDS_WORDS, st>>>(b, tab);
      else mxn::ntt_mx_dif_kernel<2><<<g, 512, (8u << 14) + 4 * mxn::C_LDS_WORDS, st>>>(b, tab);
    } else if (use_split(log_blk, (uint64_t)n_cols << (log_n - log_blk), src, out, false)) {
      if ((rc = get_table(inverse ? 1 : 0, log_blk - 1, 0, &b.tw))) return rc;
      b.tw_top = tw_b;
      b.n_units = n_cols << (log_n - log_blk);
      const dim3 grid1((b.n_units + 7) / 8 * 8 * 2);
      if (log_blk == 14) ntt16_dif_kernel<13, 1><<<grid1, 512, 8u << 13, st>>>(b);
      else ntt16_dif_kernel<12, 1><<<grid1, 256, 8u << 12, st>>>(b);
    } else {
      const dim3 grid16(1u << (log_n - log_blk), n_cols);
      if (log_blk == 12) ntt16_dif_kernel<12, 0><<<grid16, 256, 8u << 12, st>>>(b);
      else if (log_blk == 13) ntt16_dif_kernel<13, 0><<<grid16, 512, 8u << 13, st>>>(b);
      else ntt16_dif_kernel<14, 0><<<grid16, 1024, 8u << 14, st>>>(b);
    }
    BPG_LAUNCH_CHECK();
    return BP_OK;
  }
  LdsNttArgs a{};
  a.in = src; a.in_stride = src_stride; a.out = out; a.out_stride = out_stride; a.out_coset_stride = 0;
  a.tw = tw_b; a.scale = nullptr;
  a.out_scalar = inverse ? gl::inv((uint64_t)1 << log_n) : 1;
  a.log_blk = log_blk; a.log_n_total = log_n;
  dim3 grid(1u << (log_n - log_blk), n_cols, 1);
  size_t lds = (size_t)8 << log_blk;
  {
    KernelTimer kt(PROF_INTT_DIF, st, 16.0 * (double)n_cols * (double)((uint64_t)1 << log_n));
    ntt_lds_kernel<true><<<grid, lds_threads(log_blk), lds, st>>>(a);
  }
  BPG_LAUNCH_CHECK();
  return BP_OK;
}

int ntt_br2nat(const uint64_t* in, uint64_t in_stride, uint64_t* out, uint64_t out_stride, uint64_t coset_stride,
               uint32_t log_n, uint32_t n_cols, uint32_t n_cosets, const uint64_t* scale, bool inverse,
               hipStream_t st) {
  if (n_cols == 0) return BP_OK;
  const uint32_t log_blk = pick_log_blk(log_n);
  const uint64_t *tw_n = nullptr, *tw_b = nullptr;
  int rc;
  if ((rc = get_table(inverse ? 1 : 0, log_blk, 0, &tw_b))) return rc;
  if (log_blk >= 12) {
    Ntt16Args b{};
    b.in = in; b.in_stride = in_stride; b.out = out; b.out_stride = out_stride; b.out_coset_stride = coset_stride;
    b.tw = tw_b; b.scale = scale; b.out_scalar = 1; b.log_n_total = log_n; b.n_cosets = n_cosets;
    b.n_units = n_cols << (log_n - log_blk);
    {
      KernelTimer kt(PROF_LDE_DIT, st, 8.0 * (double)n_cols * (double)((uint64_t)1 << log_n) * (1.0 + n_cosets), true);
      if (use_ntt_mx(log_blk, true)) {
        const mxn::Tables* tab = nullptr;
        if ((rc = get_mx_tables(1, inverse, &tab))) return rc;
        const uint32_t g = mx_grid((b.n_units + 7) / 8 * 8 * n_cosets, log_blk);
        if (log_blk == 12) BPG_LAUNCH_TIMED(kt, mxn::ntt_mx_dit_kernel<0>, g, 256, (8u << 12) + 4 * mxn::C_LDS_WORDS, st, b, tab);
        else if (log_blk == 13) BPG_LAUNCH_TIMED(kt, mxn::ntt_mx_dit_kernel<1>, g, 512, (8u << 13) + 4 * mxn::C_LDS_WORDS, st, b, tab);
        else BPG_LAUNCH_TIMED(kt, mxn::ntt_mx_dit_kernel<2>, g, 512, (8u << 14) + 4 * mxn::C_LDS_WORDS, st, b, tab);
      } else if (use_split(log_blk, (uint64_t)b.n_units * n_cosets, in, out, true)) {
        if ((rc = get_table(inverse ? 1 : 0, log_blk - 1, 0, &b.tw))) return rc;
        b.tw_top = tw_b;
        const dim3 grid1((b.n_units + 7) / 8 * 8 * n_cosets * 2);
        if (log_blk == 14) BPG_LAUNCH_TIMED(kt, HIP_KERNEL_NAME(ntt16_dit_kernel<13, 1>), grid1, 512, 8u << 13, st, b);
        else BPG_LAUNCH_TIMED(kt, HIP_KERNEL_NAME(ntt16_dit_kernel<12, 1>), grid1, 256, 8u << 12, st, b);
      } else {
        const dim3 grid16((b.n_units + 7) / 8 * 8 * n_cosets);
        if (log_blk == 12) BPG_LAUNCH_TIMED(kt, HIP_KERNEL_NAME(ntt16_dit_kernel<12, 0>), grid16, 256, 8u << 12, st, b);
        else if (log_blk == 13) BPG_LAUNCH_TIMED(kt, HIP_KERNEL_NAME(ntt16_dit_kernel<13, 0>), grid16, 512, 8u << 13, st, b);
        else {
          const uint32_t items = grid16.x, group = 8 * n_cosets;
          const uint32_t resident = std::max<uint32_t>(group, (uint32_t)g_ntt_persist_wgs.load(std::memory_order_relaxed) / group * group);
          if (g_ntt_persist.load(std::memory_order_relaxed) && items > resident && in != out)
            BPG_LAUNCH_TIMED(kt, HIP_KERNEL_NAME(ntt16_dit_persist_kernel<14>), dim3(resident), 1024, 8u << 14, st, b, items);
          else
            BPG_LAUNCH_TIMED(kt, HIP_KERNEL_NAME(ntt16_dit_kernel<14, 0>), grid16, 1024, 8u << 14, st, b);
        }
      }
    }
    BPG_LAUNCH_CHECK();
  } else {
  LdsNttArgs a{};
  a.in = in; a.in_stride = in_stride; a.out = out; a.out_stride = out_stride; a.out_coset_stride = coset_stride;
  a.tw = tw_b; a.scale = scale; a.out_scalar = 1; a.log_blk = log_blk; a.log_n_total = log_n;
  dim3 grid(1u << (log_n - log_blk), n_cols, n_cosets);
  size_t lds = (size_t)8 << log_blk;
  {
    KernelTimer kt(PROF_LDE_DIT, st, 8.0 * (double)n_cols * (double)((uint64_t)1 << log_n) * (1.0 + n_cosets), true);
    BPG_LAUNCH_TIMED(kt, ntt_lds_kernel<false>, grid, lds_threads(log_blk), lds, st, a);
  }
  BPG_LAUNCH_CHECK();
  }
  if (log_n > LOG_BLK_MAX) {
    if ((rc = get_table(inverse ? 1 : 0, log_n, 0, &tw_n))) return rc;
    if ((rc = launch_global_passes<false>(out, out_stride, out, out_stride, coset_stride, n_cols, n_cosets, log_n,
                                          log_blk, tw_n, st)))
      return rc;
  }
  return BP_OK;
}

int bitrev_permute(uint64_t* cols, uint64_t stride, uint32_t log_n, uint32_t n_cols, hipStream_t st) {
  dim3 grid(ceil_div((uint64_t)1 << log_n, 256), n_cols);
  bitrev_permute_kernel<<<grid, 256, 0, st>>>(cols, stride, log_n);
  BPG_LAUNCH_CHECK();
  return BP_OK;
}

static int init_ntt_kernels_once() {
  BPG_HIP(hipFuncSetAttribute(reinterpret_cast<const void*>(&ntt_lds_kernel<true>),
                              hipFuncAttributeMaxDynamicSharedMemorySize, 8 << LOG_BLK_MAX));
  BPG_HIP(hipFuncSetAttribute(reinterpret_cast<const void*>(&ntt_lds_kernel<false>),
                              hipFuncAttributeMaxDynamicSharedMemorySize, 8 << LOG_BLK_MAX));
  BPG_HIP(hipFuncSetAttribute(reinterpret_cast<const void*>(&ntt16_dif_kernel<14, 0>),
                              hipFuncAttributeMaxDynamicSharedMemorySize, 8 << 14));
  BPG_HIP(hipFuncSetAttribute(reinterpret_cast<const void*>(&ntt16_dit_kernel<14, 0>),
                              hipFuncAttributeMaxDynamicSharedMemorySize, 8 << 14));
  BPG_HIP(hipFuncSetAttribute(reinterpret_cast<const void*>(&ntt16_dit_persist_kernel<14>),
                              hipFuncAttributeMaxDynamicSharedMemorySize, 8 << 14));
  BPG_HIP(hipFuncSetAttribute(reinterpret_cast<const void*>(&ntt16_dif_kernel<13, 0>),
                              hipFuncAttributeMaxDynamicSharedMemorySize, 8 << 13));
  BPG_HIP(hipFuncSetAttribute(reinterpret_cast<const void*>(&ntt16_dit_kernel<13, 0>),
                              hipFuncAttributeMaxDynamicSharedMemorySize, 8 << 13));
  BPG_HIP(hipFuncSetAttribute(reinterpret_cast<const void*>(&mxn::ntt_mx_dif_kernel<1>),
                              hipFuncAttributeMaxDynamicSharedMemorySize, (8 << 13) + 4 * mxn::C_LDS_WORDS));
  BPG_HIP(hipFuncSetAttribute(reinterpret_cast<const void*>(&mxn::ntt_mx_dif_kernel<2>),
                              hipFuncAttributeMaxDynamicSharedMemorySize, (8 << 14) + 4 * mxn::C_LDS_WORDS));
  BPG_HIP(hipFuncSetAttribute(reinterpret_cast<const void*>(&mxn::ntt_mx_dit_kernel<1>),
                              hipFuncAttributeMaxDynamicSharedMemorySize, (8 << 13) + 4 * mxn::C_LDS_WORDS));
  BPG_HIP(hipFuncSetAttribute(reinterpret_cast<const void*>(&mxn::ntt_mx_dit_kernel<2>),
                              hipFuncAttributeMaxDynamicSharedMemorySize, (8 << 14) + 4 * mxn::C_LDS_WORDS));
  BPG_HIP(hipFuncSetAttribute(reinterpret_cast<const void*>(&ntt16_dif_kernel<13, 1>),
                              hipFuncAttributeMaxDynamicSharedMemorySize, 8 << 13));
  BPG_HIP(hipFuncSetAttribute(reinterpret_cast<const void*>(&ntt16_dit_kernel<13, 1>),
                              hipFuncAttributeMaxDynamicSharedMemorySize, 8 << 13));
  return BP_OK;
}
int init_ntt_kernels() {
  static std::once_flag once;
  static int rc = BP_OK;
  std::call_once(once, [] { rc = init_ntt_kernels_once(); });
  return rc;
}

}

extern "C" {

void bp_tune_ntt_split(int mode) { bpg::g_ntt_split.store(mode); }
void bp_tune_ntt_persist(int on, int resident_workgroups) {
  bpg::g_ntt_persist.store(on != 0);
  if (resident_workgroups > 0) bpg::g_ntt_persist_wgs.store(resident_workgroups);
}
void bp_tune_ntt_mx(int mode) { bpg::g_ntt_mx.store(mode < 0 || mode > 5 ? 3 : mode); }
void bp_tune_ntt_mx_wg_per_cu(int n) { bpg::g_mx_wg_per_cu.store(n); }

int bp_debug_ntt_mx_tables(int kind, int inverse, uint8_t* out_a, int32_t* out_c, uint64_t* out_tw256,
                           uint64_t* out_tw16) try {
  if ((kind != 0 && kind != 1) || !out_a || !out_c || !out_tw256 || !out_tw16)
    return bpg::fail(BP_ERR_INVALID_INPUT, "bp_debug_ntt_mx_tables: bad argument");
  auto t = std::make_unique<mxn::Tables>();
  {
    std::lock_guard<std::mutex> lk(bpg::g_mx_mu);
    mxn::build_tables(*t, kind, inverse != 0);
  }
  memcpy(out_a, t->a, sizeof(t->a));
  memcpy(out_c, t->c, sizeof(t->c));
  memcpy(out_tw256, t->tw256, sizeof(t->tw256));
  memcpy(out_tw16, t->tw16, sizeof(t->tw16));
  return BP_OK;
}
BPG_ABI_CATCH("bp_debug_ntt_mx_tables")

int bp_ntt_batch(uint64_t* d_cols, uint32_t log_n, uint32_t n_cols, uint64_t col_stride, int dir, void* stream) try {
  if (n_cols == 0) return BP_OK;
  if (!d_cols) return bpg::fail(BP_ERR_INVALID_INPUT, "bp_ntt_batch: null buffer");
  if (log_n > 30 || col_stride < ((uint64_t)1 << log_n))
    return bpg::fail(BP_ERR_INVALID_INPUT, "bp_ntt_batch: bad shape (log_n=%u stride=%llu)", log_n,
                     (unsigned long long)col_stride);
  hipStream_t st = bpg::as_stream(stream);
  int rc;
  if ((rc = bpg::init_ntt_kernels())) return rc;
  switch (dir) {
    case BP_NTT_FWD_BR2NAT:
      return bpg::ntt_br2nat(d_cols, col_stride, d_cols, col_stride, 0, log_n, n_cols, 1, nullptr, false, st);
    case BP_NTT_INV_NAT2BR:
      return bpg::intt_nat2br(d_cols, col_stride, d_cols, col_stride, log_n, n_cols, true, st);
    case BP_NTT_FWD_NAT:
      if ((rc = bpg::bitrev_permute(d_cols, col_stride, log_n, n_cols, st))) return rc;
      return bpg::ntt_br2nat(d_cols, col_stride, d_cols, col_stride, 0, log_n, n_cols, 1, nullptr, false, st);
    case BP_NTT_INV_NAT:
      if ((rc = bpg::intt_nat2br(d_cols, col_stride, d_cols, col_stride, log_n, n_cols, true, st))) return rc;
      return bpg::bitrev_permute(d_cols, col_stride, log_n, n_cols, st);
    default:
      return bpg::fail(BP_ERR_INVALID_INPUT, "bp_ntt_batch: unknown dir %d", dir);
  }
}
BPG_ABI_CATCH("bp_ntt_batch")

int bp_intt_batch(const uint64_t* d_values, uint64_t in_stride, uint64_t* d_coeffs_out, uint64_t out_stride,
                  uint32_t log_n, uint32_t n_cols, void* stream) try {
  if (n_cols == 0) return BP_OK;
  if (!d_values || !d_coeffs_out) return bpg::fail(BP_ERR_INVALID_INPUT, "bp_intt_batch: null buffer");
  const uint64_t n = (uint64_t)1 << log_n;
  if (log_n > 30 || in_stride < n || out_stride < n) return bpg::fail(BP_ERR_INVALID_INPUT, "bp_intt_batch: bad shape (log_n=%u)", log_n);
  const uint64_t span_in = in_stride * (n_cols - 1) + n, span_out = out_stride * (n_cols - 1) + n;
  if (d_values != d_coeffs_out && d_values < d_coeffs_out + span_out && d_coeffs_out < d_values + span_in)
    return bpg::fail(BP_ERR_INVALID_INPUT, "bp_intt_batch: buffers overlap (use the same pointer for in place)");
  int rc;
  if ((rc = bpg::init_ntt_kernels())) return rc;
  return bpg::intt_nat2br(d_values, in_stride, d_coeffs_out, out_stride, log_n, n_cols, true, bpg::as_stream(stream));
}
BPG_ABI_CATCH("bp_intt_batch")

int bp_lde_batch(const uint64_t* d_in, uint64_t in_stride, uint64_t* d_coeffs_out, uint64_t coeffs_stride,
                 uint64_t* d_lde_out, uint64_t lde_stride, uint32_t log_n, uint32_t rate_bits, uint32_t n_cols,
                 int from_coeffs, void* stream) try {
  if (n_cols == 0) return BP_OK;
  const uint64_t n = (uint64_t)1 << log_n;
  if (!d_in || !d_lde_out || (!from_coeffs && !d_coeffs_out))
    return bpg::fail(BP_ERR_INVALID_INPUT, "bp_lde_batch: null buffer");
  if (log_n + rate_bits > 30 || rate_bits > 4 || in_stride < n || lde_stride < (n << rate_bits) ||
      (d_coeffs_out && coeffs_stride < n))
    return bpg::fail(BP_ERR_INVALID_INPUT, "bp_lde_batch: bad shape (log_n=%u rate_bits=%u)", log_n, rate_bits);
  if (d_coeffs_out && d_coeffs_out != d_in) {
    const uint64_t span_in = in_stride * (n_cols - 1) + n, span_c = coeffs_stride * (n_cols - 1) + n;
    if (d_in < d_coeffs_out + span_c && d_coeffs_out < d_in + span_in)
      return bpg::fail(BP_ERR_INVALID_INPUT, "bp_lde_batch: input and coefficient buffers overlap (use the same pointer for in place)");
  }
  {
    const uint64_t* src = from_coeffs ? d_in : d_coeffs_out;
    const uint64_t span_s = (from_coeffs ? in_stride : coeffs_stride) * (n_cols - 1) + n;
    const uint64_t span_l = lde_stride * (n_cols - 1) + (n << rate_bits);
    if (src < d_lde_out + span_l && d_lde_out < src + span_s)
      return bpg::fail(BP_ERR_INVALID_INPUT, "bp_lde_batch: the LDE output overlaps the coefficients it is computed from");
  }
  hipStream_t st = bpg::as_stream(stream);
  int rc;
  if ((rc = bpg::init_ntt_kernels())) return rc;
  const uint64_t* coeffs = d_in;
  uint64_t cstride = in_stride;
  if (!from_coeffs) {
    if ((rc = bpg::intt_nat2br(d_in, in_stride, d_coeffs_out, coeffs_stride, log_n, n_cols, true, st))) return rc;
    coeffs = d_coeffs_out;
    cstride = coeffs_stride;
  } else if (d_coeffs_out && d_coeffs_out != d_in) {
    BPG_HIP(hipMemcpy2DAsync(d_coeffs_out, coeffs_stride * 8, d_in, in_stride * 8, n * 8, n_cols,
                             hipMemcpyDeviceToDevice, st));
  }
  const uint64_t* scale = nullptr;
  if ((rc = bpg::get_table(2, log_n, rate_bits, &scale))) return rc;
  return bpg::ntt_br2nat(coeffs, cstride, d_lde_out, lde_stride, n, log_n, n_cols, 1u << rate_bits, scale, false,
                         st);
}
BPG_ABI_CATCH("bp_lde_batch")

}
```

Measured before the change: 34.07.

## Use shift-based power-of-two multiplies in radix-16 butterflies and inverse-NTT scaling

Adds Goldilocks multiply-by-2^k and divide-by-2^k primitives built from limb shifts plus carry-chain reduction, and uses them in a new dft16_dit path for radix-16 DIT butterflies in place of general twiddle multiplies. The 1/n output scaling of the inverse NTT is replaced by a division by 2^log_n when the scalar matches. The aim is fewer 64-bit modular multiplies in the NTT inner loops. It also enlarges the twiddle tables to the full size, disables the new path for one kernel configuration (L=14, F=0), and adds input-validation errors for unsupported direction combinations, which could break callers that used them.

```diff
diff --git a/proof_protocol_decoder_amd/csrc/gl.hpp b/proof_protocol_decoder_amd/csrc/gl.hpp
--- a/proof_protocol_decoder_amd/csrc/gl.hpp
+++ b/proof_protocol_decoder_amd/csrc/gl.hpp
@@ -231,6 +231,70 @@
 }
 #endif
 #if defined(__HIP__)
+template <int K>
+__device__ __forceinline__ void pow2_limbs(uint64_t x, uint32_t& y0, uint32_t& y1, uint32_t& y2) {
+  static_assert(K > 0 && K < 96 && (K & 31) != 0, "K = 32q + s with 0 < s < 32, q < 3");
+  constexpr int s = K & 31;
+  const uint32_t x0 = (uint32_t)x, x1 = (uint32_t)(x >> 32);
+  y0 = x0 << s;
+  y1 = (x1 << s) | (x0 >> (32 - s));
+  y2 = x1 >> (32 - s);
+}
+template <int K>
+__device__ __forceinline__ uint64_t mul_pow2(uint64_t x) {
+  uint32_t y0, y1, y2;
+  pow2_limbs<K>(x, y0, y1, y2);
+  cc::mask c, b, w, b3;
+  if constexpr (K < 32) {
+    const uint64_t V = cc::mad_eps_co(y2, cc::mk64(y0, y1), c);
+    const uint32_t lo = cc::subb0_co((uint32_t)V, c, b);
+    const uint32_t hi = cc::addc0_co((uint32_t)(V >> 32), c & ~b, w);
+    return cc::mk64(lo, hi);
+  } else if constexpr (K < 64) {
+    const uint64_t V = cc::mad_eps_co(y1, cc::mk64(0u, y0), c);
+    const uint32_t lo = cc::subb_co((uint32_t)V, y2, c, b);
+    uint32_t hi = cc::addc0_co((uint32_t)(V >> 32), c & ~b, w);
+    hi = cc::subb0_co(hi, b & ~c, w);
+    const uint32_t r0 = cc::addc0_co(lo, w, b3);
+    return cc::mk64(r0, cc::subb0_co(hi, w & ~b3, c));
+  } else {
+    const uint64_t V = (uint64_t)y0 * 0xFFFFFFFFu;
+    const uint32_t lo = cc::sub_co((uint32_t)V, y1, b);
+    const uint32_t hi = cc::subb_co((uint32_t)(V >> 32), y2, b, w);
+    const uint32_t r0 = cc::addc0_co(lo, w, b3);
+    return cc::mk64(r0, cc::subb0_co(hi, w & ~b3, c));
+  }
+}
+template <int K, int N>
+__device__ __forceinline__ void mul_pow2_n(const uint64_t (&x)[N], uint64_t (&r)[N]) {
+  static_assert(N == 3 || N == 4, "groups of 3 or 4");
+  uint32_t y0[N], y1[N], y2[N];
+#pragma unroll
+  for (int i = 0; i < N; i++) pow2_limbs<K>(x[i], y0[i], y1[i], y2[i]);
+  if constexpr (K < 32 && N == 3) cc::pow2_place_000(r, y0, y1, y2);
+  else if constexpr (K < 32) cc::pow2_place_0000(r, y0, y1, y2);
+  else if constexpr (K < 64 && N == 3) cc::pow2_place_111(r, y0, y1, y2);
+  else if constexpr (K < 64) cc::pow2_place_1111(r, y0, y1, y2);
+  else if constexpr (N == 3) cc::pow2_place_222(r, y0, y1, y2);
+  else cc::pow2_place_2222(r, y0, y1, y2);
+}
+__device__ __forceinline__ uint64_t div_pow2(uint64_t x, uint32_t k) {
+  const uint32_t y0 = (uint32_t)x << (32 - k);
+  return sub((x >> k) + y0, (uint64_t)y0 << 32);
+}
+__device__ __forceinline__ void div_pow2_n(const uint64_t (&x)[4], uint32_t k, uint64_t (&r)[4]) {
+  uint32_t y0[4], y1[4], y2[4];
+#pragma unroll
+  for (int i = 0; i < 4; i++) {
+    const uint32_t x0 = (uint32_t)x[i], x1 = (uint32_t)(x[i] >> 32);
+    y0[i] = x0 << (32 - k);
+    y1[i] = __builtin_amdgcn_alignbit(x1, x0, k);
+    y2[i] = x1 >> k;
+  }
+  cc::pow2_place_3333(r, y0, y1, y2);
+}
+#endif
+#if defined(__HIP__)
 struct DotAcc {
   uint64_t p, m, q;
   uint32_t cp, cm, cq;
diff --git a/proof_protocol_decoder_amd/csrc/gl_cc.inc b/proof_protocol_decoder_amd/csrc/gl_cc.inc
--- a/proof_protocol_decoder_amd/csrc/gl_cc.inc
+++ b/proof_protocol_decoder_amd/csrc/gl_cc.inc
@@ -218,3 +218,316 @@
       : "=&v"(x[0]), "=&v"(x[1]), "=&v"(x[2]), "=&v"(x[3]), "=&s"(co[0]), "=&s"(co[1]), "=&s"(co[2]), "=&s"(co[3])
       : "v"(a[0]), "v"(a[1]), "v"(a[2]), "v"(a[3]), "s"(ci[0]), "s"(ci[1]), "s"(ci[2]), "s"(ci[3]));
 }
+__device__ __forceinline__ void pow2_place_000(uint64_t (&r)[3], const uint32_t (&y0)[3], const uint32_t (&y1)[3], const uint32_t (&y2)[3]) {
+  uint64_t P0 = mk64(y0[0], y1[0]); mask b0, c0;
+  uint64_t P1 = mk64(y0[1], y1[1]); mask b1, c1;
+  uint64_t P2 = mk64(y0[2], y1[2]); mask b2, c2;
+  asm("v_mad_u64_u32 %0, %1, %6, -1, %0\n\tv_mad_u64_u32 %2, %3, %7, -1, %2\n\tv_mad_u64_u32 %4, %5, %8, -1, %4"
+      : "+v"(P0), "=&s"(c0), "+v"(P1), "=&s"(c1), "+v"(P2), "=&s"(c2)
+      : "v"(y2[0]), "v"(y2[1]), "v"(y2[2]));
+  uint32_t lo0 = (uint32_t)P0, hi0 = (uint32_t)(P0 >> 32);
+  uint32_t lo1 = (uint32_t)P1, hi1 = (uint32_t)(P1 >> 32);
+  uint32_t lo2 = (uint32_t)P2, hi2 = (uint32_t)(P2 >> 32);
+  asm("v_subbrev_co_u32_e64 %0, %1, 0, %0, %6\n\tv_subbrev_co_u32_e64 %2, %3, 0, %2, %7\n\tv_subbrev_co_u32_e64 %4, %5, 0, %4, %8"
+      : "+v"(lo0), "=&s"(b0), "+v"(lo1), "=&s"(b1), "+v"(lo2), "=&s"(b2)
+      : "s"(c0), "s"(c1), "s"(c2));
+  c0 &= ~b0;
+  c1 &= ~b1;
+  c2 &= ~b2;
+  asm("v_addc_co_u32_e64 %0, vcc, %0, 0, %3\n\tv_addc_co_u32_e64 %1, vcc, %1, 0, %4\n\tv_addc_co_u32_e64 %2, vcc, %2, 0, %5"
+      : "+v"(hi0), "+v"(hi1), "+v"(hi2)
+      : "s"(c0), "s"(c1), "s"(c2) : "vcc");
+  r[0] = mk64(lo0, hi0);
+  r[1] = mk64(lo1, hi1);
+  r[2] = mk64(lo2, hi2);
+}
+__device__ __forceinline__ void pow2_place_0000(uint64_t (&r)[4], const uint32_t (&y0)[4], const uint32_t (&y1)[4], const uint32_t (&y2)[4]) {
+  uint64_t P0 = mk64(y0[0], y1[0]); mask b0, c0;
+  uint64_t P1 = mk64(y0[1], y1[1]); mask b1, c1;
+  uint64_t P2 = mk64(y0[2], y1[2]); mask b2, c2;
+  uint64_t P3 = mk64(y0[3], y1[3]); mask b3, c3;
+  asm("v_mad_u64_u32 %0, %1, %8, -1, %0\n\tv_mad_u64_u32 %2, %3, %9, -1, %2\n\tv_mad_u64_u32 %4, %5, %10, -1, %4\n\tv_mad_u64_u32 %6, %7, %11, -1, %6"
+      : "+v"(P0), "=&s"(c0), "+v"(P1), "=&s"(c1), "+v"(P2), "=&s"(c2), "+v"(P3), "=&s"(c3)
+      : "v"(y2[0]), "v"(y2[1]), "v"(y2[2]), "v"(y2[3]));
+  uint32_t lo0 = (uint32_t)P0, hi0 = (uint32_t)(P0 >> 32);
+  uint32_t lo1 = (uint32_t)P1, hi1 = (uint32_t)(P1 >> 32);
+  uint32_t lo2 = (uint32_t)P2, hi2 = (uint32_t)(P2 >> 32);
+  uint32_t lo3 = (uint32_t)P3, hi3 = (uint32_t)(P3 >> 32);
+  asm("v_subbrev_co_u32_e64 %0, %1, 0, %0, %8\n\tv_subbrev_co_u32_e64 %2, %3, 0, %2, %9\n\tv_subbrev_co_u32_e64 %4, %5, 0, %4, %10\n\tv_subbrev_co_u32_e64 %6, %7, 0, %6, %11"
+      : "+v"(lo0), "=&s"(b0), "+v"(lo1), "=&s"(b1), "+v"(lo2), "=&s"(b2), "+v"(lo3), "=&s"(b3)
+      : "s"(c0), "s"(c1), "s"(c2), "s"(c3));
+  c0 &= ~b0;
+  c1 &= ~b1;
+  c2 &= ~b2;
+  c3 &= ~b3;
+  asm("v_addc_co_u32_e64 %0, vcc, %0, 0, %4\n\tv_addc_co_u32_e64 %1, vcc, %1, 0, %5\n\tv_addc_co_u32_e64 %2, vcc, %2, 0, %6\n\tv_addc_co_u32_e64 %3, vcc, %3, 0, %7"
+      : "+v"(hi0), "+v"(hi1), "+v"(hi2), "+v"(hi3)
+      : "s"(c0), "s"(c1), "s"(c2), "s"(c3) : "vcc");
+  r[0] = mk64(lo0, hi0);
+  r[1] = mk64(lo1, hi1);
+  r[2] = mk64(lo2, hi2);
+  r[3] = mk64(lo3, hi3);
+}
+__device__ __forceinline__ void pow2_place_111(uint64_t (&r)[3], const uint32_t (&y0)[3], const uint32_t (&y1)[3], const uint32_t (&y2)[3]) {
+  uint64_t P0 = mk64(0u, y0[0]); mask b0, b30, c0, w0;
+  uint64_t P1 = mk64(0u, y0[1]); mask b1, b31, c1, w1;
+  uint64_t P2 = mk64(0u, y0[2]); mask b2, b32, c2, w2;
+  asm("v_mad_u64_u32 %0, %1, %6, -1, %0\n\tv_mad_u64_u32 %2, %3, %7, -1, %2\n\tv_mad_u64_u32 %4, %5, %8, -1, %4"
+      : "+v"(P0), "=&s"(c0), "+v"(P1), "=&s"(c1), "+v"(P2), "=&s"(c2)
+      : "v"(y1[0]), "v"(y1[1]), "v"(y1[2]));
+  uint32_t lo0 = (uint32_t)P0, hi0 = (uint32_t)(P0 >> 32);
+  uint32_t lo1 = (uint32_t)P1, hi1 = (uint32_t)(P1 >> 32);
+  uint32_t lo2 = (uint32_t)P2, hi2 = (uint32_t)(P2 >> 32);
+  asm("v_subb_co_u32_e64 %0, %1, %0, %6, %7\n\tv_subb_co_u32_e64 %2, %3, %2, %8, %9\n\tv_subb_co_u32_e64 %4, %5, %4, %10, %11"
+      : "+v"(lo0), "=&s"(b0), "+v"(lo1), "=&s"(b1), "+v"(lo2), "=&s"(b2)
+      : "v"(y2[0]), "s"(c0), "v"(y2[1]), "s"(c1), "v"(y2[2]), "s"(c2));
+  const mask up0 = c0 & ~b0, dn0 = b0 & ~c0;
+  const mask up1 = c1 & ~b1, dn1 = b1 & ~c1;
+  const mask up2 = c2 & ~b2, dn2 = b2 & ~c2;
+  asm("v_addc_co_u32_e64 %0, vcc, %0, 0, %3\n\tv_addc_co_u32_e64 %1, vcc, %1, 0, %4\n\tv_addc_co_u32_e64 %2, vcc, %2, 0, %5"
+      : "+v"(hi0), "+v"(hi1), "+v"(hi2)
+      : "s"(up0), "s"(up1), "s"(up2) : "vcc");
+  asm("v_subbrev_co_u32_e64 %0, %1, 0, %0, %6\n\tv_subbrev_co_u32_e64 %2, %3, 0, %2, %7\n\tv_subbrev_co_u32_e64 %4, %5, 0, %4, %8"
+      : "+v"(hi0), "=&s"(w0), "+v"(hi1), "=&s"(w1), "+v"(hi2), "=&s"(w2)
+      : "s"(dn0), "s"(dn1), "s"(dn2));
+  asm("v_addc_co_u32_e64 %0, %1, %0, 0, %6\n\tv_addc_co_u32_e64 %2, %3, %2, 0, %7\n\tv_addc_co_u32_e64 %4, %5, %4, 0, %8"
+      : "+v"(lo0), "=&s"(b30), "+v"(lo1), "=&s"(b31), "+v"(lo2), "=&s"(b32)
+      : "s"(w0), "s"(w1), "s"(w2));
+  w0 &= ~b30;
+  w1 &= ~b31;
+  w2 &= ~b32;
+  asm("v_subbrev_co_u32_e64 %0, vcc, 0, %0, %3\n\tv_subbrev_co_u32_e64 %1, vcc, 0, %1, %4\n\tv_subbrev_co_u32_e64 %2, vcc, 0, %2, %5"
+      : "+v"(hi0), "+v"(hi1), "+v"(hi2)
+      : "s"(w0), "s"(w1), "s"(w2) : "vcc");
+  r[0] = mk64(lo0, hi0);
+  r[1] = mk64(lo1, hi1);
+  r[2] = mk64(lo2, hi2);
+}
+__device__ __forceinline__ void pow2_place_1111(uint64_t (&r)[4], const uint32_t (&y0)[4], const uint32_t (&y1)[4], const uint32_t (&y2)[4]) {
+  uint64_t P0 = mk64(0u, y0[0]); mask b0, b30, c0, w0;
+  uint64_t P1 = mk64(0u, y0[1]); mask b1, b31, c1, w1;
+  uint64_t P2 = mk64(0u, y0[2]); mask b2, b32, c2, w2;
+  uint64_t P3 = mk64(0u, y0[3]); mask b3, b33, c3, w3;
+  asm("v_mad_u64_u32 %0, %1, %8, -1, %0\n\tv_mad_u64_u32 %2, %3, %9, -1, %2\n\tv_mad_u64_u32 %4, %5, %10, -1, %4\n\tv_mad_u64_u32 %6, %7, %11, -1, %6"
+      : "+v"(P0), "=&s"(c0), "+v"(P1), "=&s"(c1), "+v"(P2), "=&s"(c2), "+v"(P3), "=&s"(c3)
+      : "v"(y1[0]), "v"(y1[1]), "v"(y1[2]), "v"(y1[3]));
+  uint32_t lo0 = (uint32_t)P0, hi0 = (uint32_t)(P0 >> 32);
+  uint32_t lo1 = (uint32_t)P1, hi1 = (uint32_t)(P1 >> 32);
+  uint32_t lo2 = (uint32_t)P2, hi2 = (uint32_t)(P2 >> 32);
+  uint32_t lo3 = (uint32_t)P3, hi3 = (uint32_t)(P3 >> 32);
+  asm("v_subb_co_u32_e64 %0, %1, %0, %8, %9\n\tv_subb_co_u32_e64 %2, %3, %2, %10, %11\n\tv_subb_co_u32_e64 %4, %5, %4, %12, %13\n\tv_subb_co_u32_e64 %6, %7, %6, %14, %15"
+      : "+v"(lo0), "=&s"(b0), "+v"(lo1), "=&s"(b1), "+v"(lo2), "=&s"(b2), "+v"(lo3), "=&s"(b3)
+      : "v"(y2[0]), "s"(c0), "v"(y2[1]), "s"(c1), "v"(y2[2]), "s"(c2), "v"(y2[3]), "s"(c3));
+  const mask up0 = c0 & ~b0, dn0 = b0 & ~c0;
+  const mask up1 = c1 & ~b1, dn1 = b1 & ~c1;
+  const mask up2 = c2 & ~b2, dn2 = b2 & ~c2;
+  const mask up3 = c3 & ~b3, dn3 = b3 & ~c3;
+  asm("v_addc_co_u32_e64 %0, vcc, %0, 0, %4\n\tv_addc_co_u32_e64 %1, vcc, %1, 0, %5\n\tv_addc_co_u32_e64 %2, vcc, %2, 0, %6\n\tv_addc_co_u32_e64 %3, vcc, %3, 0, %7"
+      : "+v"(hi0), "+v"(hi1), "+v"(hi2), "+v"(hi3)
+      : "s"(up0), "s"(up1), "s"(up2), "s"(up3) : "vcc");
+  asm("v_subbrev_co_u32_e64 %0, %1, 0, %0, %8\n\tv_subbrev_co_u32_e64 %2, %3, 0, %2, %9\n\tv_subbrev_co_u32_e64 %4, %5, 0, %4, %10\n\tv_subbrev_co_u32_e64 %6, %7, 0, %6, %11"
+      : "+v"(hi0), "=&s"(w0), "+v"(hi1), "=&s"(w1), "+v"(hi2), "=&s"(w2), "+v"(hi3), "=&s"(w3)
+      : "s"(dn0), "s"(dn1), "s"(dn2), "s"(dn3));
+  asm("v_addc_co_u32_e64 %0, %1, %0, 0, %8\n\tv_addc_co_u32_e64 %2, %3, %2, 0, %9\n\tv_addc_co_u32_e64 %4, %5, %4, 0, %10\n\tv_addc_co_u32_e64 %6, %7, %6, 0, %11"
+      : "+v"(lo0), "=&s"(b30), "+v"(lo1), "=&s"(b31), "+v"(lo2), "=&s"(b32), "+v"(lo3), "=&s"(b33)
+      : "s"(w0), "s"(w1), "s"(w2), "s"(w3));
+  w0 &= ~b30;
+  w1 &= ~b31;
+  w2 &= ~b32;
+  w3 &= ~b33;
+  asm("v_subbrev_co_u32_e64 %0, vcc, 0, %0, %4\n\tv_subbrev_co_u32_e64 %1, vcc, 0, %1, %5\n\tv_subbrev_co_u32_e64 %2, vcc, 0, %2, %6\n\tv_subbrev_co_u32_e64 %3, vcc, 0, %3, %7"
+      : "+v"(hi0), "+v"(hi1), "+v"(hi2), "+v"(hi3)
+      : "s"(w0), "s"(w1), "s"(w2), "s"(w3) : "vcc");
+  r[0] = mk64(lo0, hi0);
+  r[1] = mk64(lo1, hi1);
+  r[2] = mk64(lo2, hi2);
+  r[3] = mk64(lo3, hi3);
+}
+__device__ __forceinline__ void pow2_place_222(uint64_t (&r)[3], const uint32_t (&y0)[3], const uint32_t (&y1)[3], const uint32_t (&y2)[3]) {
+  uint64_t P0; mask b0, b30, w0;
+  uint64_t P1; mask b1, b31, w1;
+  uint64_t P2; mask b2, b32, w2;
+  asm("v_mad_u64_u32 %0, vcc, %3, -1, 0\n\tv_mad_u64_u32 %1, vcc, %4, -1, 0\n\tv_mad_u64_u32 %2, vcc, %5, -1, 0"
+      : "=&v"(P0), "=&v"(P1), "=&v"(P2)
+      : "v"(y0[0]), "v"(y0[1]), "v"(y0[2]) : "vcc");
+  uint32_t lo0 = (uint32_t)P0, hi0 = (uint32_t)(P0 >> 32);
+  uint32_t lo1 = (uint32_t)P1, hi1 = (uint32_t)(P1 >> 32);
+  uint32_t lo2 = (uint32_t)P2, hi2 = (uint32_t)(P2 >> 32);
+  asm("v_sub_co_u32_e64 %0, %1, %0, %6\n\tv_sub_co_u32_e64 %2, %3, %2, %7\n\tv_sub_co_u32_e64 %4, %5, %4, %8"
+      : "+v"(lo0), "=&s"(b0), "+v"(lo1), "=&s"(b1), "+v"(lo2), "=&s"(b2)
+      : "v"(y1[0]), "v"(y1[1]), "v"(y1[2]));
+  asm("v_subb_co_u32_e64 %0, %1, %0, %6, %7\n\tv_subb_co_u32_e64 %2, %3, %2, %8, %9\n\tv_subb_co_u32_e64 %4, %5, %4, %10, %11"
+      : "+v"(hi0), "=&s"(w0), "+v"(hi1), "=&s"(w1), "+v"(hi2), "=&s"(w2)
+      : "v"(y2[0]), "s"(b0), "v"(y2[1]), "s"(b1), "v"(y2[2]), "s"(b2));
+  asm("v_addc_co_u32_e64 %0, %1, %0, 0, %6\n\tv_addc_co_u32_e64 %2, %3, %2, 0, %7\n\tv_addc_co_u32_e64 %4, %5, %4, 0, %8"
+      : "+v"(lo0), "=&s"(b30), "+v"(lo1), "=&s"(b31), "+v"(lo2), "=&s"(b32)
+      : "s"(w0), "s"(w1), "s"(w2));
+  w0 &= ~b30;
+  w1 &= ~b31;
+  w2 &= ~b32;
+  asm("v_subbrev_co_u32_e64 %0, vcc, 0, %0, %3\n\tv_subbrev_co_u32_e64 %1, vcc, 0, %1, %4\n\tv_subbrev_co_u32_e64 %2, vcc, 0, %2, %5"
+      : "+v"(hi0), "+v"(hi1), "+v"(hi2)
+      : "s"(w0), "s"(w1), "s"(w2) : "vcc");
+  r[0] = mk64(lo0, hi0);
+  r[1] = mk64(lo1, hi1);
+  r[2] = mk64(lo2, hi2);
+}
+__device__ __forceinline__ void pow2_place_2222(uint64_t (&r)[4], const uint32_t (&y0)[4], const uint32_t (&y1)[4], const uint32_t (&y2)[4]) {
+  uint64_t P0; mask b0, b30, w0;
+  uint64_t P1; mask b1, b31, w1;
+  uint64_t P2; mask b2, b32, w2;
+  uint64_t P3; mask b3, b33, w3;
+  asm("v_mad_u64_u32 %0, vcc, %4, -1, 0\n\tv_mad_u64_u32 %1, vcc, %5, -1, 0\n\tv_mad_u64_u32 %2, vcc, %6, -1, 0\n\tv_mad_u64_u32 %3, vcc, %7, -1, 0"
+      : "=&v"(P0), "=&v"(P1), "=&v"(P2), "=&v"(P3)
+      : "v"(y0[0]), "v"(y0[1]), "v"(y0[2]), "v"(y0[3]) : "vcc");
+  uint32_t lo0 = (uint32_t)P0, hi0 = (uint32_t)(P0 >> 32);
+  uint32_t lo1 = (uint32_t)P1, hi1 = (uint32_t)(P1 >> 32);
+  uint32_t lo2 = (uint32_t)P2, hi2 = (uint32_t)(P2 >> 32);
+  uint32_t lo3 = (uint32_t)P3, hi3 = (uint32_t)(P3 >> 32);
+  asm("v_sub_co_u32_e64 %0, %1, %0, %8\n\tv_sub_co_u32_e64 %2, %3, %2, %9\n\tv_sub_co_u32_e64 %4, %5, %4, %10\n\tv_sub_co_u32_e64 %6, %7, %6, %11"
+      : "+v"(lo0), "=&s"(b0), "+v"(lo1), "=&s"(b1), "+v"(lo2), "=&s"(b2), "+v"(lo3), "=&s"(b3)
+      : "v"(y1[0]), "v"(y1[1]), "v"(y1[2]), "v"(y1[3]));
+  asm("v_subb_co_u32_e64 %0, %1, %0, %8, %9\n\tv_subb_co_u32_e64 %2, %3, %2, %10, %11\n\tv_subb_co_u32_e64 %4, %5, %4, %12, %13\n\tv_subb_co_u32_e64 %6, %7, %6, %14, %15"
+      : "+v"(hi0), "=&s"(w0), "+v"(hi1), "=&s"(w1), "+v"(hi2), "=&s"(w2), "+v"(hi3), "=&s"(w3)
+      : "v"(y2[0]), "s"(b0), "v"(y2[1]), "s"(b1), "v"(y2[2]), "s"(b2), "v"(y2[3]), "s"(b3));
+  asm("v_addc_co_u32_e64 %0, %1, %0, 0, %8\n\tv_addc_co_u32_e64 %2, %3, %2, 0, %9\n\tv_addc_co_u32_e64 %4, %5, %4, 0, %10\n\tv_addc_co_u32_e64 %6, %7, %6, 0, %11"
+      : "+v"(lo0), "=&s"(b30), "+v"(lo1), "=&s"(b31), "+v"(lo2), "=&s"(b32), "+v"(lo3), "=&s"(b33)
+      : "s"(w0), "s"(w1), "s"(w2), "s"(w3));
+  w0 &= ~b30;
+  w1 &= ~b31;
+  w2 &= ~b32;
+  w3 &= ~b33;
+  asm("v_subbrev_co_u32_e64 %0, vcc, 0, %0, %4\n\tv_subbrev_co_u32_e64 %1, vcc, 0, %1, %5\n\tv_subbrev_co_u32_e64 %2, vcc, 0, %2, %6\n\tv_subbrev_co_u32_e64 %3, vcc, 0, %3, %7"
+      : "+v"(hi0), "+v"(hi1), "+v"(hi2), "+v"(hi3)
+      : "s"(w0), "s"(w1), "s"(w2), "s"(w3) : "vcc");
+  r[0] = mk64(lo0, hi0);
+  r[1] = mk64(lo1, hi1);
+  r[2] = mk64(lo2, hi2);
+  r[3] = mk64(lo3, hi3);
+}
+__device__ __forceinline__ void pow2_place_112200(uint64_t (&r)[6], const uint32_t (&y0)[6], const uint32_t (&y1)[6], const uint32_t (&y2)[6]) {
+  uint64_t P0 = mk64(0u, y0[0]); mask b0, b30, c0, w0;
+  uint64_t P1 = mk64(0u, y0[1]); mask b1, b31, c1, w1;
+  uint64_t P2; mask b2, b32, w2;
+  uint64_t P3; mask b3, b33, w3;
+  uint64_t P4 = mk64(y0[4], y1[4]); mask b4, c4;
+  uint64_t P5 = mk64(y0[5], y1[5]); mask b5, c5;
+  asm("v_mad_u64_u32 %0, %1, %10, -1, %0\n\tv_mad_u64_u32 %2, %3, %11, -1, %2\n\tv_mad_u64_u32 %4, vcc, %12, -1, 0\n\tv_mad_u64_u32 %5, vcc, %13, -1, 0\n\tv_mad_u64_u32 %6, %7, %14, -1, %6\n\tv_mad_u64_u32 %8, %9, %15, -1, %8"
+      : "+v"(P0), "=&s"(c0), "+v"(P1), "=&s"(c1), "=&v"(P2), "=&v"(P3), "+v"(P4), "=&s"(c4), "+v"(P5), "=&s"(c5)
+      : "v"(y1[0]), "v"(y1[1]), "v"(y0[2]), "v"(y0[3]), "v"(y2[4]), "v"(y2[5]) : "vcc");
+  uint32_t lo0 = (uint32_t)P0, hi0 = (uint32_t)(P0 >> 32);
+  uint32_t lo1 = (uint32_t)P1, hi1 = (uint32_t)(P1 >> 32);
+  uint32_t lo2 = (uint32_t)P2, hi2 = (uint32_t)(P2 >> 32);
+  uint32_t lo3 = (uint32_t)P3, hi3 = (uint32_t)(P3 >> 32);
+  uint32_t lo4 = (uint32_t)P4, hi4 = (uint32_t)(P4 >> 32);
+  uint32_t lo5 = (uint32_t)P5, hi5 = (uint32_t)(P5 >> 32);
+  asm("v_subb_co_u32_e64 %0, %1, %0, %12, %13\n\tv_subb_co_u32_e64 %2, %3, %2, %14, %15\n\tv_sub_co_u32_e64 %4, %5, %4, %16\n\tv_sub_co_u32_e64 %6, %7, %6, %17\n\tv_subbrev_co_u32_e64 %8, %9, 0, %8, %18\n\tv_subbrev_co_u32_e64 %10, %11, 0, %10, %19"
+      : "+v"(lo0), "=&s"(b0), "+v"(lo1), "=&s"(b1), "+v"(lo2), "=&s"(b2), "+v"(lo3), "=&s"(b3), "+v"(lo4), "=&s"(b4), "+v"(lo5), "=&s"(b5)
+      : "v"(y2[0]), "s"(c0), "v"(y2[1]), "s"(c1), "v"(y1[2]), "v"(y1[3]), "s"(c4), "s"(c5));
+  const mask up0 = c0 & ~b0, dn0 = b0 & ~c0;
+  const mask up1 = c1 & ~b1, dn1 = b1 & ~c1;
+  c4 &= ~b4;
+  c5 &= ~b5;
+  asm("v_addc_co_u32_e64 %0, vcc, %0, 0, %8\n\tv_addc_co_u32_e64 %1, vcc, %1, 0, %9\n\tv_subb_co_u32_e64 %2, %3, %2, %10, %11\n\tv_subb_co_u32_e64 %4, %5, %4, %12, %13\n\tv_addc_co_u32_e64 %6, vcc, %6, 0, %14\n\tv_addc_co_u32_e64 %7, vcc, %7, 0, %15"
+      : "+v"(hi0), "+v"(hi1), "+v"(hi2), "=&s"(w2), "+v"(hi3), "=&s"(w3), "+v"(hi4), "+v"(hi5)
+      : "s"(up0), "s"(up1), "v"(y2[2]), "s"(b2), "v"(y2[3]), "s"(b3), "s"(c4), "s"(c5) : "vcc");
+  asm("v_subbrev_co_u32_e64 %0, %1, 0, %0, %8\n\tv_subbrev_co_u32_e64 %2, %3, 0, %2, %9\n\tv_addc_co_u32_e64 %4, %5, %4, 0, %10\n\tv_addc_co_u32_e64 %6, %7, %6, 0, %11"
+      : "+v"(hi0), "=&s"(w0), "+v"(hi1), "=&s"(w1), "+v"(lo2), "=&s"(b32), "+v"(lo3), "=&s"(b33)
+      : "s"(dn0), "s"(dn1), "s"(w2), "s"(w3));
+  w2 &= ~b32;
+  w3 &= ~b33;
+  asm("v_addc_co_u32_e64 %0, %1, %0, 0, %6\n\tv_addc_co_u32_e64 %2, %3, %2, 0, %7\n\tv_subbrev_co_u32_e64 %4, vcc, 0, %4, %8\n\tv_subbrev_co_u32_e64 %5, vcc, 0, %5, %9"
+      : "+v"(lo0), "=&s"(b30), "+v"(lo1), "=&s"(b31), "+v"(hi2), "+v"(hi3)
+      : "s"(w0), "s"(w1), "s"(w2), "s"(w3) : "vcc");
+  w0 &= ~b30;
+  w1 &= ~b31;
+  asm("v_subbrev_co_u32_e64 %0, vcc, 0, %0, %2\n\tv_subbrev_co_u32_e64 %1, vcc, 0, %1, %3"
+      : "+v"(hi0), "+v"(hi1)
+      : "s"(w0), "s"(w1) : "vcc");
+  r[0] = mk64(lo0, hi0);
+  r[1] = mk64(lo1, hi1);
+  r[2] = mk64(lo2, hi2);
+  r[3] = mk64(lo3, hi3);
+  r[4] = mk64(lo4, hi4);
+  r[5] = mk64(lo5, hi5);
+}
+__device__ __forceinline__ void pow2_place_1112200(uint64_t (&r)[7], const uint32_t (&y0)[7], const uint32_t (&y1)[7], const uint32_t (&y2)[7]) {
+  uint64_t P0 = mk64(0u, y0[0]); mask b0, b30, c0, w0;
+  uint64_t P1 = mk64(0u, y0[1]); mask b1, b31, c1, w1;
+  uint64_t P2 = mk64(0u, y0[2]); mask b2, b32, c2, w2;
+  uint64_t P3; mask b3, b33, w3;
+  uint64_t P4; mask b4, b34, w4;
+  uint64_t P5 = mk64(y0[5], y1[5]); mask b5, c5;
+  uint64_t P6 = mk64(y0[6], y1[6]); mask b6, c6;
+  asm("v_mad_u64_u32 %0, %1, %12, -1, %0\n\tv_mad_u64_u32 %2, %3, %13, -1, %2\n\tv_mad_u64_u32 %4, %5, %14, -1, %4\n\tv_mad_u64_u32 %6, vcc, %15, -1, 0\n\tv_mad_u64_u32 %7, vcc, %16, -1, 0\n\tv_mad_u64_u32 %8, %9, %17, -1, %8\n\tv_mad_u64_u32 %10, %11, %18, -1, %10"
+      : "+v"(P0), "=&s"(c0), "+v"(P1), "=&s"(c1), "+v"(P2), "=&s"(c2), "=&v"(P3), "=&v"(P4), "+v"(P5), "=&s"(c5), "+v"(P6), "=&s"(c6)
+      : "v"(y1[0]), "v"(y1[1]), "v"(y1[2]), "v"(y0[3]), "v"(y0[4]), "v"(y2[5]), "v"(y2[6]) : "vcc");
+  uint32_t lo0 = (uint32_t)P0, hi0 = (uint32_t)(P0 >> 32);
+  uint32_t lo1 = (uint32_t)P1, hi1 = (uint32_t)(P1 >> 32);
+  uint32_t lo2 = (uint32_t)P2, hi2 = (uint32_t)(P2 >> 32);
+  uint32_t lo3 = (uint32_t)P3, hi3 = (uint32_t)(P3 >> 32);
+  uint32_t lo4 = (uint32_t)P4, hi4 = (uint32_t)(P4 >> 32);
+  uint32_t lo5 = (uint32_t)P5, hi5 = (uint32_t)(P5 >> 32);
+  uint32_t lo6 = (uint32_t)P6, hi6 = (uint32_t)(P6 >> 32);
+  asm("v_subb_co_u32_e64 %0, %1, %0, %14, %15\n\tv_subb_co_u32_e64 %2, %3, %2, %16, %17\n\tv_subb_co_u32_e64 %4, %5, %4, %18, %19\n\tv_sub_co_u32_e64 %6, %7, %6, %20\n\tv_sub_co_u32_e64 %8, %9, %8, %21\n\tv_subbrev_co_u32_e64 %10, %11, 0, %10, %22\n\tv_subbrev_co_u32_e64 %12, %13, 0, %12, %23"
+      : "+v"(lo0), "=&s"(b0), "+v"(lo1), "=&s"(b1), "+v"(lo2), "=&s"(b2), "+v"(lo3), "=&s"(b3), "+v"(lo4), "=&s"(b4), "+v"(lo5), "=&s"(b5), "+v"(lo6), "=&s"(b6)
+      : "v"(y2[0]), "s"(c0), "v"(y2[1]), "s"(c1), "v"(y2[2]), "s"(c2), "v"(y1[3]), "v"(y1[4]), "s"(c5), "s"(c6));
+  const mask up0 = c0 & ~b0, dn0 = b0 & ~c0;
+  const mask up1 = c1 & ~b1, dn1 = b1 & ~c1;
+  const mask up2 = c2 & ~b2, dn2 = b2 & ~c2;
+  c5 &= ~b5;
+  c6 &= ~b6;
+  asm("v_addc_co_u32_e64 %0, vcc, %0, 0, %9\n\tv_addc_co_u32_e64 %1, vcc, %1, 0, %10\n\tv_addc_co_u32_e64 %2, vcc, %2, 0, %11\n\tv_subb_co_u32_e64 %3, %4, %3, %12, %13\n\tv_subb_co_u32_e64 %5, %6, %5, %14, %15\n\tv_addc_co_u32_e64 %7, vcc, %7, 0, %16\n\tv_addc_co_u32_e64 %8, vcc, %8, 0, %17"
+      : "+v"(hi0), "+v"(hi1), "+v"(hi2), "+v"(hi3), "=&s"(w3), "+v"(hi4), "=&s"(w4), "+v"(hi5), "+v"(hi6)
+      : "s"(up0), "s"(up1), "s"(up2), "v"(y2[3]), "s"(b3), "v"(y2[4]), "s"(b4), "s"(c5), "s"(c6) : "vcc");
+  asm("v_subbrev_co_u32_e64 %0, %1, 0, %0, %10\n\tv_subbrev_co_u32_e64 %2, %3, 0, %2, %11\n\tv_subbrev_co_u32_e64 %4, %5, 0, %4, %12\n\tv_addc_co_u32_e64 %6, %7, %6, 0, %13\n\tv_addc_co_u32_e64 %8, %9, %8, 0, %14"
+      : "+v"(hi0), "=&s"(w0), "+v"(hi1), "=&s"(w1), "+v"(hi2), "=&s"(w2), "+v"(lo3), "=&s"(b33), "+v"(lo4), "=&s"(b34)
+      : "s"(dn0), "s"(dn1), "s"(dn2), "s"(w3), "s"(w4));
+  w3 &= ~b33;
+  w4 &= ~b34;
+  asm("v_addc_co_u32_e64 %0, %1, %0, 0, %8\n\tv_addc_co_u32_e64 %2, %3, %2, 0, %9\n\tv_addc_co_u32_e64 %4, %5, %4, 0, %10\n\tv_subbrev_co_u32_e64 %6, vcc, 0, %6, %11\n\tv_subbrev_co_u32_e64 %7, vcc, 0, %7, %12"
+      : "+v"(lo0), "=&s"(b30), "+v"(lo1), "=&s"(b31), "+v"(lo2), "=&s"(b32), "+v"(hi3), "+v"(hi4)
+      : "s"(w0), "s"(w1), "s"(w2), "s"(w3), "s"(w4) : "vcc");
+  w0 &= ~b30;
+  w1 &= ~b31;
+  w2 &= ~b32;
+  asm("v_subbrev_co_u32_e64 %0, vcc, 0, %0, %3\n\tv_subbrev_co_u32_e64 %1, vcc, 0, %1, %4\n\tv_subbrev_co_u32_e64 %2, vcc, 0, %2, %5"
+      : "+v"(hi0), "+v"(hi1), "+v"(hi2)
+      : "s"(w0), "s"(w1), "s"(w2) : "vcc");
+  r[0] = mk64(lo0, hi0);
+  r[1] = mk64(lo1, hi1);
+  r[2] = mk64(lo2, hi2);
+  r[3] = mk64(lo3, hi3);
+  r[4] = mk64(lo4, hi4);
+  r[5] = mk64(lo5, hi5);
+  r[6] = mk64(lo6, hi6);
+}
+__device__ __forceinline__ void pow2_place_3333(uint64_t (&r)[4], const uint32_t (&y0)[4], const uint32_t (&y1)[4], const uint32_t (&y2)[4]) {
+  uint32_t lo0 = y1[0], hi0 = y2[0]; mask b30, c0, w0;
+  uint32_t lo1 = y1[1], hi1 = y2[1]; mask b31, c1, w1;
+  uint32_t lo2 = y1[2], hi2 = y2[2]; mask b32, c2, w2;
+  uint32_t lo3 = y1[3], hi3 = y2[3]; mask b33, c3, w3;
+  asm("v_add_co_u32_e64 %0, %1, %0, %8\n\tv_add_co_u32_e64 %2, %3, %2, %9\n\tv_add_co_u32_e64 %4, %5, %4, %10\n\tv_add_co_u32_e64 %6, %7, %6, %11"
+      : "+v"(lo0), "=&s"(c0), "+v"(lo1), "=&s"(c1), "+v"(lo2), "=&s"(c2), "+v"(lo3), "=&s"(c3)
+      : "v"(y0[0]), "v"(y0[1]), "v"(y0[2]), "v"(y0[3]));
+  asm("v_addc_co_u32_e64 %0, vcc, %0, 0, %4\n\tv_addc_co_u32_e64 %1, vcc, %1, 0, %5\n\tv_addc_co_u32_e64 %2, vcc, %2, 0, %6\n\tv_addc_co_u32_e64 %3, vcc, %3, 0, %7"
+      : "+v"(hi0), "+v"(hi1), "+v"(hi2), "+v"(hi3)
+      : "s"(c0), "s"(c1), "s"(c2), "s"(c3) : "vcc");
+  asm("v_sub_co_u32_e64 %0, %1, %0, %8\n\tv_sub_co_u32_e64 %2, %3, %2, %9\n\tv_sub_co_u32_e64 %4, %5, %4, %10\n\tv_sub_co_u32_e64 %6, %7, %6, %11"
+      : "+v"(hi0), "=&s"(w0), "+v"(hi1), "=&s"(w1), "+v"(hi2), "=&s"(w2), "+v"(hi3), "=&s"(w3)
+      : "v"(y0[0]), "v"(y0[1]), "v"(y0[2]), "v"(y0[3]));
+  asm("v_addc_co_u32_e64 %0, %1, %0, 0, %8\n\tv_addc_co_u32_e64 %2, %3, %2, 0, %9\n\tv_addc_co_u32_e64 %4, %5, %4, 0, %10\n\tv_addc_co_u32_e64 %6, %7, %6, 0, %11"
+      : "+v"(lo0), "=&s"(b30), "+v"(lo1), "=&s"(b31), "+v"(lo2), "=&s"(b32), "+v"(lo3), "=&s"(b33)
+      : "s"(w0), "s"(w1), "s"(w2), "s"(w3));
+  w0 &= ~b30;
+  w1 &= ~b31;
+  w2 &= ~b32;
+  w3 &= ~b33;
+  asm("v_subbrev_co_u32_e64 %0, vcc, 0, %0, %4\n\tv_subbrev_co_u32_e64 %1, vcc, 0, %1, %5\n\tv_subbrev_co_u32_e64 %2, vcc, 0, %2, %6\n\tv_subbrev_co_u32_e64 %3, vcc, 0, %3, %7"
+      : "+v"(hi0), "+v"(hi1), "+v"(hi2), "+v"(hi3)
+      : "s"(w0), "s"(w1), "s"(w2), "s"(w3) : "vcc");
+  r[0] = mk64(lo0, hi0);
+  r[1] = mk64(lo1, hi1);
+  r[2] = mk64(lo2, hi2);
+  r[3] = mk64(lo3, hi3);
+}
diff --git a/proof_protocol_decoder_amd/csrc/ntt.hip b/proof_protocol_decoder_amd/csrc/ntt.hip
--- a/proof_protocol_decoder_amd/csrc/ntt.hip
+++ b/proof_protocol_decoder_amd/csrc/ntt.hip
@@ -12,81 +12,161 @@
 
 constexpr uint32_t LOG_BLK_MAX = 14;
 
-template <int N>
-__device__ __forceinline__ void mul_group(uint64_t (&x)[16], const int (&idx)[4], const uint64_t (&d)[4], const uint64_t (&w)[4]) {
-  if constexpr (N == 4) {
-    uint64_t r[4];
-    gl::mul_n<4>(d, w, r);
-#pragma unroll
-    for (int i = 0; i < 4; i++) x[idx[i]] = r[i];
-  } else if constexpr (N == 3) {
-    const uint64_t d3[3] = {d[0], d[1], d[2]}, w3[3] = {w[0], w[1], w[2]};
-    uint64_t r[3];
-    gl::mul_n<3>(d3, w3, r);
-#pragma unroll
-    for (int i = 0; i < 3; i++) x[idx[i]] = r[i];
-  } else {
-#pragma unroll
-    for (int i = 0; i < N; i++) x[idx[i]] = gl::mul(d[i], w[i]);
-  }
+
+__device__ constexpr int W16_K[16] = {0, 60, 24, 84, 48, 12, 72, 36, 0, 60, 24, 84, 48, 12, 72, 36};
+__device__ constexpr bool W16_NEG[16] = {0, 1, 1, 0, 0, 0, 1, 1, 1, 0, 0, 1, 1, 1, 0, 0};
+template <bool DIF, int S>
+__device__ constexpr int dft16_e(int m) {
+  return DIF ? (16 - ((m & ((8 >> S) - 1)) << S)) & 15 : ((m & ((1 << S) - 1)) << (3 - S)) & 15;
+}
+template <bool DIF, int S>
+__device__ constexpr int dft16_count(int q) {
+  int n = 0;
+  for (int m = 0; m < 16; m++) {
+    if (m & (DIF ? 8 >> S : 1 << S)) continue;
+    const int e = dft16_e<DIF, S>(m);
+    if ((e & 7) && (q < 0 || W16_K[e] / 32 == q)) n++;
+  }
+  return n;
+}
+template <int K>
+__device__ __forceinline__ void limbs_if(int k, uint64_t v, uint32_t& y0, uint32_t& y1, uint32_t& y2) {
+  if (k == K) gl::pow2_limbs<K>(v, y0, y1, y2);
+}
+template <bool DIF, int S>
+__device__ __forceinline__ void dft16_shift_mults(uint64_t (&x)[16]) {
+  constexpr int span = DIF ? 8 >> S : 1 << S, NM = dft16_count<DIF, S>(-1);
+  if constexpr (NM > 0) {
+    static_assert((NM == 4 && dft16_count<DIF, S>(1) == 4) ||
+                  (NM == 6 && dft16_count<DIF, S>(1) == 2 && dft16_count<DIF, S>(2) == 2) ||
+                  (NM == 7 && dft16_count<DIF, S>(1) == 3 && dft16_count<DIF, S>(2) == 2), "group signature");
+    uint32_t y0[NM], y1[NM], y2[NM];
+    uint64_t r[NM];
+    int pos[NM], n = 0;
+    constexpr int order[3] = {1, 2, 0};
+#pragma unroll
+    for (int c = 0; c < 3; c++) {
+#pragma unroll
+      for (int m = 0; m < 16; m++) {
+        if (m & span) continue;
+        const int e = dft16_e<DIF, S>(m), k = W16_K[e];
+        if (!(e & 7) || k / 32 != order[c]) continue;
+        const uint64_t v = x[m + span];
+        limbs_if<12>(k, v, y0[n], y1[n], y2[n]); limbs_if<24>(k, v, y0[n], y1[n], y2[n]);
+        limbs_if<36>(k, v, y0[n], y1[n], y2[n]); limbs_if<48>(k, v, y0[n], y1[n], y2[n]);
+        limbs_if<60>(k, v, y0[n], y1[n], y2[n]); limbs_if<72>(k, v, y0[n], y1[n], y2[n]);
+        limbs_if<84>(k, v, y0[n], y1[n], y2[n]);
+        pos[n++] = m + span;
+      }
+    }
+    if constexpr (NM == 4) gl::cc::pow2_place_1111(r, y0, y1, y2);
+    else if constexpr (NM == 6) gl::cc::pow2_place_112200(r, y0, y1, y2);
+    else gl::cc::pow2_place_1112200(r, y0, y1, y2);
+#pragma unroll
+    for (int i = 0; i < NM; i++) x[pos[i]] = r[i];
+  }
+}
+template <bool EARLY>
+__device__ __forceinline__ void dft16_twiddle_layer(uint64_t (&x)[16], const uint64_t* __restrict__ tw, uint32_t j,
+                                                    uint32_t tw_shift) {
+  constexpr uint32_t BR4[16] = {0, 8, 4, 12, 2, 10, 6, 14, 1, 9, 5, 13, 3, 11, 7, 15};
+  uint64_t tv[16];
+  if constexpr (EARLY) {
+#pragma unroll
+    for (int m = 1; m < 16; m++) tv[m] = tw[(j * BR4[m]) << tw_shift];
+  }
+#pragma unroll
+  for (int m0 = 0; m0 < 16; m0 += 4) {
+    if constexpr (!EARLY) {
+#pragma unroll
+      for (int i = (m0 ? 0 : 1); i < 4; i++) tv[m0 + i] = tw[(j * BR4[m0 + i]) << tw_shift];
+    }
+    if (m0 == 0) {
+      const uint64_t v[3] = {x[1], x[2], x[3]}, w[3] = {tv[1], tv[2], tv[3]};
+      uint64_t r[3];
+      gl::mul_n<3>(v, w, r);
+#pragma unroll
+      for (int i = 0; i < 3; i++) x[1 + i] = r[i];
+    } else {
+      uint64_t v[4], w[4], r[4];
+#pragma unroll
+      for (int i = 0; i < 4; i++) {
+        v[i] = x[m0 + i];
+        w[i] = tv[m0 + i];
+      }
+      gl::mul_n<4>(v, w, r);
+#pragma unroll
+      for (int i = 0; i < 4; i++) x[m0 + i] = r[i];
+    }
+    __builtin_amdgcn_sched_barrier(0);
+  }
+}
+template <bool DIF, int S>
+__device__ __forceinline__ void dft16_adds(uint64_t (&x)[16]) {
+  constexpr int span = DIF ? 8 >> S : 1 << S;
+#pragma unroll
+  for (int k0 = 0; k0 < 8; k0 += 4) {
+    uint64_t p[4], q[4], sum[4], dif[4];
+#pragma unroll
+    for (int i = 0; i < 4; i++) {
+      const int k = k0 + i, m = (k / span) * 2 * span + (k % span);
+      const bool swap = DIF && W16_NEG[dft16_e<DIF, S>(m)];
+      p[i] = swap ? x[m + span] : x[m];
+      q[i] = swap ? x[m] : x[m + span];
+    }
+    gl::canon_n<4>(q);
+    gl::add_n<4>(p, q, sum);
+    gl::sub_n<4>(p, q, dif);
+#pragma unroll
+    for (int i = 0; i < 4; i++) {
+      const int k = k0 + i, m = (k / span) * 2 * span + (k % span);
+      const bool swap = !DIF && W16_NEG[dft16_e<DIF, S>(m)];
+      x[m] = swap ? dif[i] : sum[i];
+      x[m + span] = swap ? sum[i] : dif[i];
+    }
+  }
+}
+template <int S>
+__device__ __forceinline__ void dft16_dif_stage(uint64_t (&x)[16]) {
+  dft16_adds<true, S>(x);
+  dft16_shift_mults<true, S>(x);
+  __builtin_amdgcn_sched_barrier(0);
+}
+template <int S>
+__device__ __forceinline__ void dft16_dit_stage(uint64_t (&x)[16]) {
+  dft16_shift_mults<false, S>(x);
+  dft16_adds<false, S>(x);
+  __builtin_amdgcn_sched_barrier(0);
+}
+template <bool J0>
+__device__ __forceinline__ void dft16_dif(uint64_t (&x)[16], const uint64_t* __restrict__ tw, uint32_t j, uint32_t tw_shift) {
+  dft16_dif_stage<0>(x);
+  dft16_dif_stage<1>(x);
+  dft16_dif_stage<2>(x);
+  dft16_dif_stage<3>(x);
+  if constexpr (!J0) dft16_twiddle_layer<false>(x, tw, j, tw_shift);
+}
+template <bool J0>
+__device__ __forceinline__ void dft16_dit(uint64_t (&x)[16], const uint64_t* __restrict__ tw, uint32_t j, uint32_t tw_shift) {
+  if constexpr (!J0) dft16_twiddle_layer<true>(x, tw, j, tw_shift);
+  dft16_dit_stage<0>(x);
+  dft16_dit_stage<1>(x);
+  dft16_dit_stage<2>(x);
+  dft16_dit_stage<3>(x);
 }
 
 template <int LOGR, bool J0 = false>
 __device__ __forceinline__ void dif_butterflies(uint64_t (&x)[1 << LOGR], const uint64_t* __restrict__ tw,
                                                 uint32_t j, uint32_t log_sub, uint32_t tw_shift) {
   constexpr int R = 1 << LOGR, NB = R / 2;
+  if constexpr (LOGR == 4) {
+    dft16_dif<J0>(x, tw, j, tw_shift);
+    return;
+  }
 #pragma unroll
   for (int s = 0; s < LOGR; s++) {
     const int half = R >> (s + 1);
-    if constexpr (NB % 4 == 0 && J0 && LOGR == 4) {
-      uint64_t dd[NB];
-#pragma unroll
-      for (int k0 = 0; k0 < NB; k0 += 4) {
-        uint64_t a[4], b[4], d[4], r[4];
-#pragma unroll
-        for (int i = 0; i < 4; i++) {
-          const int k = k0 + i, m = (k / half) * 2 * half + (k % half);
-          a[i] = x[m];
-          b[i] = x[m + half];
-        }
-        gl::canon_n<4>(b);
-        gl::add_n<4>(a, b, r);
-        gl::sub_n<4>(a, b, d);
-#pragma unroll
-        for (int i = 0; i < 4; i++) {
-          const int k = k0 + i, m = (k / half) * 2 * half + (k % half);
-          x[m] = r[i];
-          dd[k] = d[i];
-        }
-      }
-      int cnt = 0;
-      int idx[4] = {0, 0, 0, 0};
-      uint64_t dv[4] = {0, 0, 0, 0}, wv[4] = {0, 0, 0, 0};
-      uint64_t xx[16];
-#pragma unroll
-      for (int i = 0; i < 16; i++) xx[i] = x[i];
-#pragma unroll
-      for (int k = 0; k < NB; k++) {
-        const int m = (k / half) * 2 * half + (k % half), e = m & (half - 1);
-        if (e == 0) {
-          xx[m + half] = dd[k];
-        } else {
-          idx[cnt] = m + half;
-          dv[cnt] = dd[k];
-          wv[cnt] = tw[(uint32_t)e << (tw_shift + s)];
-          cnt++;
-          if (cnt == 4) {
-            mul_group<4>(xx, idx, dv, wv);
-            cnt = 0;
-          }
-        }
-      }
-      if (cnt == 3) mul_group<3>(xx, idx, dv, wv);
-      else if (cnt == 2) mul_group<2>(xx, idx, dv, wv);
-      else if (cnt == 1) mul_group<1>(xx, idx, dv, wv);
-#pragma unroll
-      for (int i = 0; i < 16; i++) x[i] = xx[i];
-    } else if constexpr (NB % 4 == 0) {
+    if constexpr (NB % 4 == 0) {
 #pragma unroll
       for (int k0 = 0; k0 < NB; k0 += 4) {
         uint64_t a[4], b[4], d[4], w[4], r[4];
@@ -130,57 +210,18 @@
     }
   }
 }
-template <int LOGR, bool J0 = false>
+template <int LOGR, bool J0 = false, bool CT = true>
 __device__ __forceinline__ void dit_butterflies(uint64_t (&x)[1 << LOGR], const uint64_t* __restrict__ tw,
                                                 uint32_t j, uint32_t log_sub, uint32_t tw_shift) {
   constexpr int R = 1 << LOGR, NB = R / 2;
+  if constexpr (LOGR == 4 && CT) {
+    dft16_dit<J0>(x, tw, j, tw_shift);
+    return;
+  }
 #pragma unroll
   for (int s = 0; s < LOGR; s++) {
     const int step = 1 << s;
-    if constexpr (NB % 4 == 0 && J0 && LOGR == 4) {
-      uint64_t xx[16];
-#pragma unroll
-      for (int i = 0; i < 16; i++) xx[i] = x[i];
-      int cnt = 0;
-      int idx[4] = {0, 0, 0, 0};
-      uint64_t dv[4] = {0, 0, 0, 0}, wv[4] = {0, 0, 0, 0};
-#pragma unroll
-      for (int k = 0; k < NB; k++) {
-        const int m = (k / step) * 2 * step + (k % step), e = m & (step - 1);
-        if (e != 0) {
-          idx[cnt] = m + step;
-          dv[cnt] = x[m + step];
-          wv[cnt] = tw[(uint32_t)e << (tw_shift + (LOGR - 1 - s))];
-          cnt++;
-          if (cnt == 4) {
-            mul_group<4>(xx, idx, dv, wv);
-            cnt = 0;
-          }
-        }
-      }
-      if (cnt == 3) mul_group<3>(xx, idx, dv, wv);
-      else if (cnt == 2) mul_group<2>(xx, idx, dv, wv);
-      else if (cnt == 1) mul_group<1>(xx, idx, dv, wv);
-#pragma unroll
-      for (int k0 = 0; k0 < NB; k0 += 4) {
-        uint64_t a[4], r[4], hi[4], lo[4];
-#pragma unroll
-        for (int i = 0; i < 4; i++) {
-          const int k = k0 + i, m = (k / step) * 2 * step + (k % step);
-          a[i] = xx[m];
-          r[i] = xx[m + step];
-        }
-        gl::canon_n<4>(r);
-        gl::add_n<4>(a, r, hi);
-        gl::sub_n<4>(a, r, lo);
-#pragma unroll
-        for (int i = 0; i < 4; i++) {
-          const int k = k0 + i, m = (k / step) * 2 * step + (k % step);
-          x[m] = hi[i];
-          x[m + step] = lo[i];
-        }
-      }
-    } else if constexpr (NB % 4 == 0) {
+    if constexpr (NB % 4 == 0) {
 #pragma unroll
       for (int k0 = 0; k0 < NB; k0 += 4) {
         uint64_t a[4], v[4], w[4], r[4], hi[4], lo[4];
@@ -247,6 +288,7 @@
   const uint64_t* tw;
   const uint64_t* scale;
   uint64_t out_scalar;
+  uint32_t out_log;
   uint32_t log_blk;
   uint32_t log_n_total;
 };
@@ -285,7 +327,9 @@
       __syncthreads();
     }
   }
-  if (DIF && a.out_scalar != 1) {
+  if (DIF && a.out_log) {
+    for (uint32_t i = threadIdx.x; i < n; i += blockDim.x) dst[i] = gl::canon(gl::div_pow2(buf[i], a.out_log));
+  } else if (DIF && a.out_scalar != 1) {
     for (uint32_t i = threadIdx.x; i < n; i += blockDim.x) dst[i] = gl::mulc(buf[i], a.out_scalar);
   } else {
     for (uint32_t i = threadIdx.x; i < n; i += blockDim.x) dst[i] = gl::canon(buf[i]);
@@ -331,6 +375,7 @@
   const uint64_t* tw;
   const uint64_t* scale;
   uint64_t out_scalar;
+  uint32_t out_log;
   uint32_t log_n_total, n_cosets, n_units;
   const uint64_t* tw_top;
 };
@@ -402,7 +447,18 @@
 #pragma unroll
   for (int m = 0; m < 16; m++) buf[swz<L>(base | m)] = x[m];
   __syncthreads();
-  if (a.out_scalar != 1) {
+  if (a.out_log) {
+#pragma unroll
+    for (int m0 = 0; m0 < 16; m0 += 4) {
+      uint64_t v[4], r[4];
+#pragma unroll
+      for (int i = 0; i < 4; i++) v[i] = buf[swz<L>((m0 + i) * T + t)];
+      gl::div_pow2_n(v, a.out_log, r);
+      gl::canon_n<4>(r);
+#pragma unroll
+      for (int i = 0; i < 4; i++) dst[(m0 + i) * T + t] = r[i];
+    }
+  } else if (a.out_scalar != 1) {
 #pragma unroll
     for (int m0 = 0; m0 < 16; m0 += 4) {
       uint64_t v[4], w[4], r[4];
@@ -435,6 +491,7 @@
   extern __shared__ uint64_t buf[];
   constexpr uint32_t T = (1u << L) / 16;
   constexpr int RT = (L % 4 == 0) ? 4 : (L % 4);
+  constexpr bool CT = !(L == 14 && F == 0);
   const uint32_t id = blockIdx.x, k = id >> 3;
   const uint32_t per = a.n_cosets << F;
   const uint32_t ch = k % per, coset = ch >> F, h = F ? (ch & 1) : 0, unit = (k / per) * 8 + (id & 7);
@@ -517,7 +574,7 @@
   for (int b = 4; b + 4 <= L - RT; b += 4) {
 #pragma unroll
     for (int m = 0; m < 16; m++) x[m] = buf[swz<L>(insert4(t, m, b))];
-    dit_butterflies<4>(x, tw, t & ((1u << b) - 1), b, L - (b + 4));
+    dit_butterflies<4, false, CT>(x, tw, t & ((1u << b) - 1), b, L - (b + 4));
 #pragma unroll
     for (int m = 0; m < 16; m++) buf[swz<L>(insert4(t, m, b))] = x[m];
     __syncthreads();
@@ -610,7 +667,7 @@
       asm volatile("" : "+v"(tc));
 #pragma unroll
       for (int m = 0; m < 16; m++) x[m] = buf[swz<L>(insert4(tc, m, b))];
-      dit_butterflies<4>(x, tw, tc & ((1u << b) - 1), b, L - (b + 4));
+      dit_butterflies<4, false, false>(x, tw, tc & ((1u << b) - 1), b, L - (b + 4));
 #pragma unroll
       for (int m = 0; m < 16; m++) buf[swz<L>(insert4(tc, m, b))] = x[m];
       __syncthreads();
@@ -794,7 +851,7 @@
     dim3 grid(ceil_div((uint64_t)1 << log_n, 256), 1u << rate_bits);
     coset_scale_table_kernel<<<grid, 256, 0, 0>>>(d, log_n, rate_bits, gl::root(log_n + rate_bits), kind == 3);
   } else {
-    uint32_t count = log_n ? (1u << (log_n - 1)) : 1;
+    uint32_t count = 1u << log_n;
     BPG_HIP(hipMalloc(&d, (uint64_t)count * 8));
     uint64_t w = gl::root(log_n);
     if (kind == 1) w = gl::inv(w);
@@ -883,6 +940,11 @@
   if (mode == 2) return true;
   if (dit) return mode == 3 && log_blk == 13 && workgroups < 512;
   return log_blk == 14 || workgroups < 512;
+}
+
+static uint32_t pow2_inverse_log(uint64_t scalar, uint32_t k) {
+  if (k < 1 || k > 31) return 0;
+  return gl::mulc(scalar, (uint64_t)1 << k) == 1 && gl::canon(scalar) == gl::P - gl::pow(2, 96 - k) ? k : 0;
 }
 
 static uint32_t lds_threads(uint32_t log_blk) {
@@ -929,6 +991,7 @@
 int intt_nat2br(const uint64_t* in, uint64_t in_stride, uint64_t* out, uint64_t out_stride, uint32_t log_n,
                 uint32_t n_cols, bool inverse, hipStream_t st) {
   if (n_cols == 0) return BP_OK;
+  if (!inverse) return fail(BP_ERR_INVALID_INPUT, "intt_nat2br: the natural -> bit-reversed transform exists for the inverse root only");
   const uint32_t log_blk = pick_log_blk(log_n);
   const uint64_t *tw_n = nullptr, *tw_b = nullptr;
   int rc;
@@ -945,6 +1008,7 @@
     Ntt16Args b{};
     b.in = src; b.in_stride = src_stride; b.out = out; b.out_stride = out_stride; b.out_coset_stride = 0;
     b.tw = tw_b; b.scale = nullptr; b.out_scalar = inverse ? gl::inv((uint64_t)1 << log_n) : 1;
+    b.out_log = inverse ? pow2_inverse_log(b.out_scalar, log_n) : 0;
     b.log_n_total = log_n; b.n_cosets = 1; b.n_units = 0;
     KernelTimer kt(PROF_INTT_DIF, st, 16.0 * (double)n_cols * (double)((uint64_t)1 << log_n));
     if (use_ntt_mx(log_blk, false)) {
@@ -975,6 +1039,7 @@
   a.in = src; a.in_stride = src_stride; a.out = out; a.out_stride = out_stride; a.out_coset_stride = 0;
   a.tw = tw_b; a.scale = nullptr;
   a.out_scalar = inverse ? gl::inv((uint64_t)1 << log_n) : 1;
+  a.out_log = inverse ? pow2_inverse_log(a.out_scalar, log_n) : 0;
   a.log_blk = log_blk; a.log_n_total = log_n;
   dim3 grid(1u << (log_n - log_blk), n_cols, 1);
   size_t lds = (size_t)8 << log_blk;
@@ -990,6 +1055,7 @@
                uint32_t log_n, uint32_t n_cols, uint32_t n_cosets, const uint64_t* scale, bool inverse,
                hipStream_t st) {
   if (n_cols == 0) return BP_OK;
+  if (inverse) return fail(BP_ERR_INVALID_INPUT, "ntt_br2nat: the bit-reversed -> natural transform exists for the forward root only");
   const uint32_t log_blk = pick_log_blk(log_n);
   const uint64_t *tw_n = nullptr, *tw_b = nullptr;
   int rc;
```

Result: no change. 34.18 (median of 6 runs) (+0.3%).
